# knagrecha/saturn

Hardware: AMD Instinct MI355X
Metric: samples_per_s (higher is better)
Workload: dtype bf16; 1 GPU; model=gptj-6b, global_batch=16, seq_len=512, parallelism=dp1, optimizer=fused_sgd

## Files before the change

### saturn_amd/executors/megatron.py

```python

from __future__ import annotations

from timeit import default_timer as timer
from typing import Any, Dict, List, Optional, Tuple

from saturn_amd.core.technique import BaseTechnique
from saturn_amd.executors.launch import (
    destroy_process_group,
    gang_spawn,
    init_process_group,
)

TRIAL_BATCHES = 3


def _tp_worker(rank: int, world: int, task, tid: int, batch_count: int,
               params: Optional[Dict[str, Any]], trial: bool):
    import torch
    import torch.distributed as dist

    from saturn_amd.executors.ddp import _make_optimizer
    from saturn_amd.parallel.tensor import (
        tp_full_state_dict,
        tp_resync_replicated,
        tp_shard_model,
    )

    backend = init_process_group(rank, world)
    try:
        device = (
            torch.device("cuda", rank) if backend == "nccl" else torch.device("cpu")
        )
        dtype = torch.bfloat16 if backend == "nccl" else torch.float32
        from saturn_amd.executors.ddp import build_model_on

        model = build_model_on(task, device, dtype)
        model.train()
        if world > 1:
            with torch.no_grad():
                for p in model.parameters():
                    dist.broadcast(p.data, src=0)
        model = tp_shard_model(model)
        optimizer = _make_optimizer(task, model)

        import os as _os

        opt_path = _os.path.join(
            task.save_dir, f"{task.name}.tpopt.w{world}.r{rank}.pt"
        )
        if not trial and _os.path.isfile(opt_path):
            try:
                optimizer.load_state_dict(
                    torch.load(opt_path, map_location="cpu", weights_only=False)
                )
            except Exception:
                pass

        it = task.get_iterator() if not trial else task.get_fresh_iterator()

        def next_batch():
            nonlocal it
            try:
                return next(it)
            except StopIteration:
                it = task.get_fresh_iterator()
                return next(it)

        def step(batch):
            x, y = batch
            x = x.to(device, non_blocking=True)
            y = y.to(device, non_blocking=True)
            if x.is_floating_point():
                x = x.to(dtype)
            loss = task.loss_function(model(x), y)
            loss.backward()
            optimizer.step()
            optimizer.zero_grad(set_to_none=True)

        if trial:
            step(next_batch())
            if device.type == "cuda":
                torch.cuda.synchronize()
                torch.cuda.reset_peak_memory_stats()
            t0 = timer()
            for _ in range(TRIAL_BATCHES - 1):
                step(next_batch())
            if device.type == "cuda":
                torch.cuda.synchronize()
            hbm = (
                torch.cuda.max_memory_allocated() / 2**30
                if device.type == "cuda"
                else 0.0
            )
            return ((timer() - t0) / (TRIAL_BATCHES - 1), hbm)
        RESYNC_EVERY = 64
        for i in range(batch_count):
            step(next_batch())
            if (i + 1) % RESYNC_EVERY == 0:
                tp_resync_replicated(model)
        if device.type == "cuda":
            torch.cuda.synchronize()
        tp_resync_replicated(model)
        sd = tp_full_state_dict(model)
        if rank == 0 and sd is not None:
            task.save_checkpoint(sd, None)
        if _os.environ.get("SATURN_SKIP_CKPT") != "1":
            tmp = opt_path + ".tmp"
            torch.save(optimizer.state_dict(), tmp)
            _os.replace(tmp, opt_path)
        if world > 1:
            dist.barrier()
        return None
    finally:
        destroy_process_group()


class MegatronExecutor(BaseTechnique):

    name = "megatron"

    @staticmethod
    def execute(task, gpus: List[int], tid: int, batch_count: int) -> None:
        params = (
            task.selected_strategy.parameters
            if task.selected_strategy is not None
            else {}
        )
        gang_spawn(_tp_worker, len(gpus), tid, task, tid, batch_count, params, False)

    @staticmethod
    def search(
        task, gpus: List[int], tid: int
    ) -> Tuple[Optional[Dict[str, Any]], float]:
        if len(gpus) < 2:
            return None, float("inf")
        try:
            out = gang_spawn(
                _tp_worker, len(gpus), tid, task, tid, TRIAL_BATCHES,
                {"tp": len(gpus)}, True,
            )
        except Exception:
            return None, float("inf")
        if out is None:
            return None, float("inf")
        bt, hbm = out
        return dict(tp=len(gpus), hbm_peak_gb=round(hbm, 2)), bt
```

### saturn_amd/models/gptj.py

```python

from __future__ import annotations


import os
from dataclasses import dataclass

import torch
import torch.nn as nn

from saturn_amd.ops.functional import (
    fused_gelu,
    FusedLayerNorm,
    apply_rope,
    causal_attention,
    fused_add3,
    fused_cross_entropy,
    rope_tables,
    FusedDropout,
    FusedEmbedding,
    gptj_mlp,
    mlp_fused_supported,
    gptj_branches,
    gptj_branches_supported,
)


@dataclass
class GPTJConfig:
    vocab_size: int = 50400
    n_ctx: int = 512
    n_embd: int = 4096
    n_head: int = 16
    n_layer: int = 28
    rotary_dim: int = 64
    embd_pdrop: float = 0.0
    resid_pdrop: float = 0.0


class GPTJAttention(nn.Module):
    def __init__(self, cfg: GPTJConfig):
        super().__init__()
        self.n_head = cfg.n_head
        self.head_dim = cfg.n_embd // cfg.n_head
        self.rotary_dim = cfg.rotary_dim
        E = cfg.n_embd
        self.q_proj = nn.Linear(E, E, bias=False)
        self.k_proj = nn.Linear(E, E, bias=False)
        self.v_proj = nn.Linear(E, E, bias=False)
        self.out_proj = nn.Linear(E, E, bias=False)
        self.n_ctx = cfg.n_ctx
        self._rope_f32 = rope_tables(cfg.n_ctx, cfg.rotary_dim)

    def _rope(self, device):
        if self._rope_f32[0].device != device:
            self._rope_f32 = tuple(t.to(device) for t in self._rope_f32)
        return self._rope_f32

    def forward(self, x):
        B, T, E = x.shape
        H, D = self.n_head, self.head_dim
        q = self.q_proj(x).view(B, T, H, D)
        k = self.k_proj(x).view(B, T, H, D)
        v = self.v_proj(x).view(B, T, H, D)
        cos, sin = self._rope(x.device)
        q = apply_rope(q, cos, sin)
        k = apply_rope(k, cos, sin)
        q = q.transpose(1, 2)
        k = k.transpose(1, 2)
        v = v.transpose(1, 2)
        o = causal_attention(q, k, v)
        o = o.transpose(1, 2).reshape(B, T, -1)
        return self.out_proj(o)


class GPTJMLP(nn.Module):
    def __init__(self, cfg: GPTJConfig):
        super().__init__()
        E = cfg.n_embd
        self.fc_in = nn.Linear(E, 4 * E)
        self.fc_out = nn.Linear(4 * E, E)

    @staticmethod
    def _plain_linear(m) -> bool:
        return type(m) is nn.Linear and not (
            m._forward_hooks
            or m._forward_pre_hooks
            or m._backward_hooks
            or m._backward_pre_hooks
        )

    def _use_fused(self, x) -> bool:
        if os.environ.get("SAMD_MLP_FUSED", "1") == "0":
            return False
        fi, fo = self.fc_in, self.fc_out
        return (
            x.is_cuda
            and self._plain_linear(fi)
            and self._plain_linear(fo)
            and mlp_fused_supported(x, fi.weight, fi.bias, fo.weight, fo.bias)
        )

    def forward(self, x):
        if self._use_fused(x):
            fi, fo = self.fc_in, self.fc_out
            return gptj_mlp(x, fi.weight, fi.bias, fo.weight, fo.bias)
        return self.fc_out(fused_gelu(self.fc_in(x)))


class GPTJBlock(nn.Module):

    def __init__(self, cfg: GPTJConfig):
        super().__init__()
        self.ln_1 = FusedLayerNorm(cfg.n_embd)
        self.attn = GPTJAttention(cfg)
        self.mlp = GPTJMLP(cfg)
        self.drop = FusedDropout(cfg.resid_pdrop)

    @staticmethod
    def _hooked(m) -> bool:
        return bool(
            m._forward_hooks
            or m._forward_pre_hooks
            or m._backward_hooks
            or m._backward_pre_hooks
        )

    def _use_fused(self, h) -> bool:
        if (os.environ.get("SAMD_MLP_FUSED", "1") == "0"
                or os.environ.get("SAMD_BLOCK_FUSED", "1") == "0"):
            return False
        attn, mlp = self.attn, self.mlp
        if type(attn) is not GPTJAttention or type(mlp) is not GPTJMLP:
            return False
        if not (h.is_cuda and h.dtype == torch.bfloat16 and h.dim() == 3):
            return False
        if self.drop.p != 0.0:
            return False
        from saturn_amd.parallel.sequence import sp_world

        if sp_world() != 1:
            return False
        if any(self._hooked(m) for b in (attn, mlp, self.drop) for m in b.modules()):
            return False
        projs = (attn.q_proj, attn.k_proj, attn.v_proj, attn.out_proj)
        fi, fo = mlp.fc_in, mlp.fc_out
        if not all(GPTJMLP._plain_linear(m) for m in (*projs, fi, fo)):
            return False
        E = h.shape[-1]
        if any(m.bias is not None or m.weight.shape != (E, E)
               or m.weight.dtype != torch.bfloat16 or not m.weight.is_cuda
               for m in projs):
            return False
        return mlp_fused_supported(
            h, fi.weight, fi.bias, fo.weight, fo.bias
        ) and gptj_branches_supported(
            h, attn.n_head, attn.rotary_dim, attn._rope_f32[0].shape[0]
        )

    def forward(self, x):
        h = self.ln_1(x)
        if self._use_fused(h):
            attn, mlp = self.attn, self.mlp
            cos, sin = attn._rope(h.device)
            a, m = gptj_branches(
                h, attn.q_proj.weight, attn.k_proj.weight, attn.v_proj.weight,
                attn.out_proj.weight, mlp.fc_in.weight, mlp.fc_in.bias,
                mlp.fc_out.weight, mlp.fc_out.bias, cos, sin, attn.n_head,
            )
            return fused_add3(x, a, m)
        return fused_add3(x, self.drop(self.attn(h)), self.drop(self.mlp(h)))


class GPTJForCausalLM(nn.Module):
    def __init__(self, cfg: GPTJConfig):
        super().__init__()
        self.cfg = cfg
        self.wte = FusedEmbedding(cfg.vocab_size, cfg.n_embd)
        self.drop = FusedDropout(cfg.embd_pdrop)
        self.h = nn.ModuleList(GPTJBlock(cfg) for _ in range(cfg.n_layer))
        self.ln_f = FusedLayerNorm(cfg.n_embd)
        self.lm_head = nn.Linear(cfg.n_embd, cfg.vocab_size, bias=True)
        self.apply(self._init)

    @staticmethod
    def _init(m):
        if isinstance(m, nn.Linear):
            nn.init.normal_(m.weight, std=0.02)
            if m.bias is not None:
                nn.init.zeros_(m.bias)
        elif isinstance(m, nn.Embedding):
            nn.init.normal_(m.weight, std=0.02)

    def forward(self, input_ids):
        x = self.drop(self.wte(input_ids))
        for block in self.h:
            x = block(x)
        x = self.ln_f(x)
        return self.lm_head(x)


def pretraining_loss(logits, labels):
    return fused_cross_entropy(logits, labels, shift=True)


class _EmbedStage(nn.Module):
    def __init__(self, wte):
        super().__init__()
        self.wte = wte

    def forward(self, input_ids):
        return self.wte(input_ids)


class _HeadStage(nn.Module):
    def __init__(self, ln_f, lm_head):
        super().__init__()
        self.ln_f = ln_f
        self.lm_head = lm_head

    def forward(self, x):
        return self.lm_head(self.ln_f(x))


def as_sequential(model: GPTJForCausalLM) -> nn.Sequential:
    return nn.Sequential(
        _EmbedStage(model.wte), *model.h, _HeadStage(model.ln_f, model.lm_head)
    )


def get_gptj_model(kwargs=None):
    kwargs = kwargs or {}
    cfg = GPTJConfig(
        n_layer=kwargs.get("n_layer", 28),
        n_embd=kwargs.get("n_embd", 4096),
        n_head=kwargs.get("n_head", 16),
        n_ctx=kwargs.get("n_ctx", 512),
        vocab_size=kwargs.get("vocab_size", 50400),
        rotary_dim=kwargs.get("rotary_dim", 64),
        embd_pdrop=kwargs.get("embd_pdrop", 0.0),
        resid_pdrop=kwargs.get("resid_pdrop", 0.0),
    )
    torch.manual_seed(kwargs.get("seed", 0))
    return GPTJForCausalLM(cfg)


class SyntheticTokens(torch.utils.data.Dataset):

    def __init__(self, n: int, seq_len: int, vocab: int, seed: int = 1):
        g = torch.Generator().manual_seed(seed)
        self.data = torch.randint(0, vocab, (n, seq_len), generator=g)

    def __len__(self):
        return len(self.data)

    def __getitem__(self, i):
        return self.data[i]


def _collate(batch):
    x = torch.stack(batch)
    return x, x.clone()


def make_token_dataloader(batch_size=8, seq_len=512, vocab=50400, n_batches=64):
    def get_dataloader():
        return torch.utils.data.DataLoader(
            SyntheticTokens(batch_size * n_batches, seq_len, vocab),
            batch_size=batch_size,
            shuffle=False,
            collate_fn=_collate,
        )

    return get_dataloader
```

### saturn_amd/ops/csrc/bindings.cpp

```cpp

#include <torch/extension.h>
#include <vector>

namespace samd {
void fused_sgd(std::vector<at::Tensor> params, std::vector<at::Tensor> grads,
               std::vector<at::Tensor> moms, std::vector<at::Tensor> masters,
               double lr, double momentum, double weight_decay);
void fused_adam(std::vector<at::Tensor> params, std::vector<at::Tensor> grads,
                std::vector<at::Tensor> ms, std::vector<at::Tensor> vs,
                std::vector<at::Tensor> masters, double lr, double beta1,
                double beta2, double eps, double weight_decay, double bc1,
                double bc2);
std::vector<at::Tensor> norm_fwd(at::Tensor x, at::Tensor w,
                                 c10::optional<at::Tensor> b, double eps,
                                 bool rms);
std::vector<at::Tensor> norm_bwd(at::Tensor dy, at::Tensor x, at::Tensor w,
                                 at::Tensor mean, at::Tensor rstd, bool rms,
                                 bool needs_db);
std::vector<at::Tensor> ce_fwd(at::Tensor logits, at::Tensor targets,
                               int64_t Tr, int64_t ignore_index);
at::Tensor ce_bwd(at::Tensor logits, at::Tensor targets, at::Tensor lse,
                  at::Tensor dloss, int64_t Tr, int64_t ignore_index);
void rope_apply(at::Tensor y, at::Tensor x, at::Tensor cos_t, at::Tensor sin_t,
                int64_t t_len, int64_t t_off, bool half_style, bool backward);
at::Tensor gelu_fwd(at::Tensor x);
at::Tensor gelu_bwd(at::Tensor dy, at::Tensor x);
std::vector<at::Tensor> attn_fwd(at::Tensor q, at::Tensor k, at::Tensor v,
                                 bool causal, int64_t kv_len);
std::vector<at::Tensor> attn_bwd(at::Tensor dout, at::Tensor q, at::Tensor k,
                                 at::Tensor v, at::Tensor o, at::Tensor lse,
                                 bool causal, int64_t kv_len);
std::string attn_dispatch(int64_t T, int64_t D);
at::Tensor add3(at::Tensor a, at::Tensor b, at::Tensor c);
at::Tensor swiglu_fwd(at::Tensor gate, at::Tensor up);
std::vector<at::Tensor> swiglu_bwd(at::Tensor dout, at::Tensor gate,
                                   at::Tensor up);
at::Tensor embed_fwd(at::Tensor weight, at::Tensor idx);
at::Tensor embed_bwd(at::Tensor dout, at::Tensor idx, long vocab);
at::Tensor dropout_fwd(at::Tensor x, double p, long seed);
at::Tensor dropout_bwd(at::Tensor dout, double p, long seed);
std::vector<at::Tensor> moe_route_fwd(at::Tensor logits, int64_t top_k,
                                      at::ScalarType out_dtype);
at::Tensor moe_route_bwd(at::Tensor logits, at::Tensor ids,
                         at::Tensor dweights);
std::vector<at::Tensor> moe_sort(at::Tensor ids, int64_t n_expert);
at::Tensor moe_permute_fwd(at::Tensor x, at::Tensor order, int64_t top_k);
at::Tensor moe_permute_bwd(at::Tensor dxs, at::Tensor pos);
at::Tensor moe_combine_fwd(at::Tensor y, at::Tensor weights, at::Tensor pos);
std::vector<at::Tensor> moe_combine_bwd(at::Tensor dout, at::Tensor y,
                                        at::Tensor weights, at::Tensor pos);
std::vector<at::Tensor> mlp_act_bwd(at::Tensor d_act, at::Tensor pre,
                                    bool want_dT, bool want_aT);
std::vector<at::Tensor> transpose_colsum(at::Tensor x, bool want_sum);
std::vector<at::Tensor> mlp_bwd(at::Tensor g, at::Tensor h, at::Tensor pre,
                                at::Tensor W_in, at::Tensor W_out,
                                bool use_tn_in, bool use_tn_out);
void transpose_into(at::Tensor x, at::Tensor dst);
at::Tensor rope_bwd_t(at::Tensor dy, at::Tensor cos_t, at::Tensor sin_t,
                      int64_t t_len, int64_t t_off, int64_t dim,
                      at::Tensor dxT);
std::vector<at::Tensor> gptj_branches_bwd(
    at::Tensor g_a, at::Tensor g_m, at::Tensor h, at::Tensor pre, at::Tensor q,
    at::Tensor k, at::Tensor v, at::Tensor o, at::Tensor lse, at::Tensor Wq,
    at::Tensor Wk, at::Tensor Wv, at::Tensor Wo, at::Tensor W_in,
    at::Tensor W_out, at::Tensor cos_t, at::Tensor sin_t, int64_t t_off,
    bool tn_in, bool tn_out, bool tn_qkv, bool tn_o, bool dh_accum);
}

PYBIND11_MODULE(TORCH_EXTENSION_NAME, m) {
  m.doc() = "saturn_amd hand-written CDNA4 (gfx950) kernels";
  m.def("fused_sgd", &samd::fused_sgd, "fused multi-tensor SGD");
  m.def("fused_adam", &samd::fused_adam, "fused multi-tensor AdamW");
  m.def("norm_fwd", &samd::norm_fwd, "LayerNorm/RMSNorm forward");
  m.def("norm_bwd", &samd::norm_bwd, "LayerNorm/RMSNorm backward");
  m.def("ce_fwd", &samd::ce_fwd, "fused cross-entropy forward");
  m.def("ce_bwd", &samd::ce_bwd, "fused cross-entropy backward");
  m.def("rope_apply", &samd::rope_apply,
        "fused rotary embedding (out-of-place, offset table rows)");
  m.def("gelu_fwd", &samd::gelu_fwd, "fused tanh-approx GELU forward");
  m.def("gelu_bwd", &samd::gelu_bwd, "fused tanh-approx GELU backward");
  m.def("attn_fwd", &samd::attn_fwd, "fused flash attention forward",
        py::arg("q"), py::arg("k"), py::arg("v"), py::arg("causal"),
        py::arg("kv_len") = -1);
  m.def("attn_dispatch", &samd::attn_dispatch,
        "kernel instantiations attn_fwd/attn_bwd launch for (padded T, D)",
        py::arg("T"), py::arg("D"));
  m.def("attn_bwd", &samd::attn_bwd, "fused flash attention backward",
        py::arg("dout"), py::arg("q"), py::arg("k"), py::arg("v"),
        py::arg("o"), py::arg("lse"), py::arg("causal"),
        py::arg("kv_len") = -1);
  m.def("add3", &samd::add3, "fused 3-way residual add");
  m.def("swiglu_fwd", &samd::swiglu_fwd, "fused silu(gate)*up");
  m.def("swiglu_bwd", &samd::swiglu_bwd, "fused SwiGLU backward");
  m.def("embed_fwd", &samd::embed_fwd, "token embedding gather");
  m.def("embed_bwd", &samd::embed_bwd, "embedding scatter-add backward");
  m.def("dropout_fwd", &samd::dropout_fwd, "counter-based fused dropout");
  m.def("dropout_bwd", &samd::dropout_bwd, "dropout backward (mask recompute)");
  m.def("moe_route_fwd", &samd::moe_route_fwd,
        "MoE softmax + top-k + renormalise (ties to the lower expert)");
  m.def("moe_route_bwd", &samd::moe_route_bwd, "MoE routing backward");
  m.def("moe_sort", &samd::moe_sort,
        "stable counting sort of (token, slot) pairs by expert");
  m.def("moe_permute_fwd", &samd::moe_permute_fwd,
        "gather token rows into expert order");
  m.def("moe_permute_bwd", &samd::moe_permute_bwd,
        "sum each token's k permuted rows");
  m.def("moe_combine_fwd", &samd::moe_combine_fwd,
        "weighted sum of each token's k expert rows");
  m.def("moe_combine_bwd", &samd::moe_combine_bwd,
        "combine backward: dy and fp32 dweights");
  m.def("mlp_act_bwd", &samd::mlp_act_bwd,
        "GELU backward + transposed d_pre / gelu(pre) + fp32 bias grad",
        py::arg("d_act"), py::arg("pre"), py::arg("want_dT") = true,
        py::arg("want_aT") = true);
  m.def("transpose_colsum", &samd::transpose_colsum,
        "bf16 transpose with optional fp32 column sums");
  m.def("mlp_bwd", &samd::mlp_bwd,
        "GPT-J MLP backward with TN-layout weight gradients");
  m.def("transpose_into", &samd::transpose_into,
        "bf16 transpose stored into a caller-given [N, M] view",
        py::arg("x"), py::arg("dst"));
  m.def("rope_bwd_t", &samd::rope_bwd_t,
        "interleaved RoPE backward that also stores dx^T into a [E, M] view",
        py::arg("dy"), py::arg("cos"), py::arg("sin"), py::arg("t_len"),
        py::arg("t_off"), py::arg("dim"), py::arg("dxT"));
  m.def("gptj_branches_bwd", &samd::gptj_branches_bwd,
        "GPT-J attention + MLP branch backward with shared transposes");
}
```

### saturn_amd/ops/csrc/fused_optim.hip

```cpp

#include <torch/extension.h>
#include <ATen/hip/HIPContext.h>
#include <vector>

#include "common.h"

namespace samd {

constexpr int MAX_T = 32;
constexpr int GRP = 8;

typedef __attribute__((ext_vector_type(8))) short short8v_;
typedef __attribute__((ext_vector_type(4))) float float4v_;

struct SgdArgs {
  void* p[MAX_T];
  void* g[MAX_T];
  void* m[MAX_T];
  void* w[MAX_T];
  long cum[MAX_T + 1];
  long numel[MAX_T];
  int n_tensors;
  float lr, momentum, weight_decay;
};

template <typename T, bool HAS_M, bool HAS_W>
__device__ __forceinline__ void sgd_elem(T* p, const T* g, float* m, float* w,
                                         long j, const SgdArgs& a) {
  float pv = HAS_W ? w[j] : toF<T>(p[j]);
  float gv = toF<T>(g[j]);
  if (a.weight_decay != 0.f) gv += a.weight_decay * pv;
  if (HAS_M) {
    float mv = m[j] * a.momentum + gv;
    m[j] = mv;
    gv = mv;
  }
  float nv = pv - a.lr * gv;
  if (HAS_W) w[j] = nv;
  p[j] = fromF<T>(nv);
}

template <typename T, bool HAS_M, bool HAS_W>
__global__ void fused_sgd_kernel(SgdArgs a) {
  const long total = a.cum[a.n_tensors];
  const long stride = (long)gridDim.x * blockDim.x;
  for (long i = blockIdx.x * (long)blockDim.x + threadIdx.x; i < total;
       i += stride) {
    int t = 0;
#pragma unroll
    for (int k = 0; k < MAX_T; ++k)
      if (k < a.n_tensors && i >= a.cum[k + 1]) t = k + 1;
    const long grp = i - a.cum[t];
    const long base = grp * GRP;
    T* p = reinterpret_cast<T*>(a.p[t]);
    const T* g = reinterpret_cast<const T*>(a.g[t]);
    float* m = HAS_M ? reinterpret_cast<float*>(a.m[t]) : nullptr;
    float* w = HAS_W ? reinterpret_cast<float*>(a.w[t]) : nullptr;
    const long n = a.numel[t];
    if constexpr (sizeof(T) == 2) {
      if (base + GRP <= n) {
        short8v_ pv = *reinterpret_cast<short8v_*>(p + base);
        short8v_ gv = *reinterpret_cast<const short8v_*>(g + base);
        float4v_ m0, m1, w0, w1;
        if (HAS_M) {
          m0 = *reinterpret_cast<float4v_*>(m + base);
          m1 = *reinterpret_cast<float4v_*>(m + base + 4);
        }
        if (HAS_W) {
          w0 = *reinterpret_cast<float4v_*>(w + base);
          w1 = *reinterpret_cast<float4v_*>(w + base + 4);
        }
#pragma unroll
        for (int e = 0; e < GRP; ++e) {
          T pe, ge;
          pe.x = (unsigned short)pv[e];
          ge.x = (unsigned short)gv[e];
          float pf = HAS_W ? (e < 4 ? w0[e] : w1[e - 4]) : toF<T>(pe);
          float gf = toF<T>(ge);
          if (a.weight_decay != 0.f) gf += a.weight_decay * pf;
          if (HAS_M) {
            float mv = (e < 4 ? m0[e] : m1[e - 4]) * a.momentum + gf;
            if (e < 4) m0[e] = mv; else m1[e - 4] = mv;
            gf = mv;
          }
          float nf = pf - a.lr * gf;
          if (HAS_W) {
            if (e < 4) w0[e] = nf; else w1[e - 4] = nf;
          }
          T out = fromF<T>(nf);
          pv[e] = (short)out.x;
        }
        *reinterpret_cast<short8v_*>(p + base) = pv;
        if (HAS_M) {
          *reinterpret_cast<float4v_*>(m + base) = m0;
          *reinterpret_cast<float4v_*>(m + base + 4) = m1;
        }
        if (HAS_W) {
          *reinterpret_cast<float4v_*>(w + base) = w0;
          *reinterpret_cast<float4v_*>(w + base + 4) = w1;
        }
      } else {
        for (long j = base; j < n; ++j)
          sgd_elem<T, HAS_M, HAS_W>(p, g, m, w, j, a);
      }
    } else {
      const long end = (base + GRP <= n) ? base + GRP : n;
      for (long j = base; j < end; ++j)
        sgd_elem<T, HAS_M, HAS_W>(p, g, m, w, j, a);
    }
  }
}

struct AdamArgs {
  void* p[MAX_T];
  void* g[MAX_T];
  void* m[MAX_T];
  void* v[MAX_T];
  void* w[MAX_T];
  long cum[MAX_T + 1];
  long numel[MAX_T];
  int n_tensors;
  float lr, beta1, beta2, eps, weight_decay, bc1, bc2;
};

template <typename T, bool HAS_W>
__device__ __forceinline__ void adam_elem(T* p, const T* g, float* m, float* v,
                                          float* w, long j, const AdamArgs& a,
                                          float inv_bc1, float inv_bc2) {
  float gv = toF<T>(g[j]);
  float mv = a.beta1 * m[j] + (1.f - a.beta1) * gv;
  float vv = a.beta2 * v[j] + (1.f - a.beta2) * gv * gv;
  m[j] = mv;
  v[j] = vv;
  float denom = sqrtf(vv * inv_bc2) + a.eps;
  float upd = (mv * inv_bc1) / denom;
  float pv = HAS_W ? w[j] : toF<T>(p[j]);
  if (a.weight_decay != 0.f) pv *= (1.f - a.lr * a.weight_decay);
  float nv = pv - a.lr * upd;
  if (HAS_W) w[j] = nv;
  p[j] = fromF<T>(nv);
}

template <typename T, bool HAS_W>
__global__ void fused_adam_kernel(AdamArgs a) {
  const long total = a.cum[a.n_tensors];
  const long stride = (long)gridDim.x * blockDim.x;
  const float inv_bc1 = 1.f / a.bc1;
  const float inv_bc2 = 1.f / a.bc2;
  for (long i = blockIdx.x * (long)blockDim.x + threadIdx.x; i < total;
       i += stride) {
    int t = 0;
#pragma unroll
    for (int k = 0; k < MAX_T; ++k)
      if (k < a.n_tensors && i >= a.cum[k + 1]) t = k + 1;
    const long grp = i - a.cum[t];
    const long base = grp * GRP;
    T* p = reinterpret_cast<T*>(a.p[t]);
    const T* g = reinterpret_cast<const T*>(a.g[t]);
    float* m = reinterpret_cast<float*>(a.m[t]);
    float* v = reinterpret_cast<float*>(a.v[t]);
    float* w = HAS_W ? reinterpret_cast<float*>(a.w[t]) : nullptr;
    const long n = a.numel[t];
    if constexpr (sizeof(T) == 2) {
      if (base + GRP <= n) {
        short8v_ pv = *reinterpret_cast<short8v_*>(p + base);
        short8v_ gv = *reinterpret_cast<const short8v_*>(g + base);
        float4v_ m0 = *reinterpret_cast<float4v_*>(m + base);
        float4v_ m1 = *reinterpret_cast<float4v_*>(m + base + 4);
        float4v_ v0 = *reinterpret_cast<float4v_*>(v + base);
        float4v_ v1 = *reinterpret_cast<float4v_*>(v + base + 4);
        float4v_ w0, w1;
        if (HAS_W) {
          w0 = *reinterpret_cast<float4v_*>(w + base);
          w1 = *reinterpret_cast<float4v_*>(w + base + 4);
        }
#pragma unroll
        for (int e = 0; e < GRP; ++e) {
          T ge;
          ge.x = (unsigned short)gv[e];
          float gf = toF<T>(ge);
          float mv = a.beta1 * (e < 4 ? m0[e] : m1[e - 4]) + (1.f - a.beta1) * gf;
          float vv = a.beta2 * (e < 4 ? v0[e] : v1[e - 4]) + (1.f - a.beta2) * gf * gf;
          if (e < 4) { m0[e] = mv; v0[e] = vv; } else { m1[e-4] = mv; v1[e-4] = vv; }
          float denom = sqrtf(vv * inv_bc2) + a.eps;
          float upd = (mv * inv_bc1) / denom;
          T pe;
          pe.x = (unsigned short)pv[e];
          float pf = HAS_W ? (e < 4 ? w0[e] : w1[e - 4]) : toF<T>(pe);
          if (a.weight_decay != 0.f) pf *= (1.f - a.lr * a.weight_decay);
          float nf = pf - a.lr * upd;
          if (HAS_W) {
            if (e < 4) w0[e] = nf; else w1[e - 4] = nf;
          }
          T out = fromF<T>(nf);
          pv[e] = (short)out.x;
        }
        *reinterpret_cast<short8v_*>(p + base) = pv;
        *reinterpret_cast<float4v_*>(m + base) = m0;
        *reinterpret_cast<float4v_*>(m + base + 4) = m1;
        *reinterpret_cast<float4v_*>(v + base) = v0;
        *reinterpret_cast<float4v_*>(v + base + 4) = v1;
        if (HAS_W) {
          *reinterpret_cast<float4v_*>(w + base) = w0;
          *reinterpret_cast<float4v_*>(w + base + 4) = w1;
        }
      } else {
        for (long j = base; j < n; ++j)
          adam_elem<T, HAS_W>(p, g, m, v, w, j, a, inv_bc1, inv_bc2);
      }
    } else {
      const long end = (base + GRP <= n) ? base + GRP : n;
      for (long j = base; j < end; ++j)
        adam_elem<T, HAS_W>(p, g, m, v, w, j, a, inv_bc1, inv_bc2);
    }
  }
}

static int grid_for(long total, int block) {
  long g = (total + block - 1) / block;
  return (int)std::min<long>(std::max<long>(g, 1), 4096);
}

static long groups_of(long numel) { return (numel + GRP - 1) / GRP; }

template <typename scalar_t>
static void sgd_launch(std::vector<at::Tensor>& params,
                       std::vector<at::Tensor>& grads,
                       std::vector<at::Tensor>& moms,
                       std::vector<at::Tensor>& masters, double lr,
                       double momentum, double weight_decay) {
  auto stream = at::hip::getCurrentHIPStream();
  const bool has_m = !moms.empty();
  const bool has_w = !masters.empty();
  for (size_t base = 0; base < params.size(); base += MAX_T) {
    SgdArgs a{};
    a.n_tensors = (int)std::min<size_t>(MAX_T, params.size() - base);
    a.lr = (float)lr;
    a.momentum = (float)momentum;
    a.weight_decay = (float)weight_decay;
    long cum = 0;
    a.cum[0] = 0;
    for (int k = 0; k < a.n_tensors; ++k) {
      a.p[k] = params[base + k].data_ptr();
      a.g[k] = grads[base + k].data_ptr();
      a.m[k] = has_m ? moms[base + k].data_ptr() : nullptr;
      a.w[k] = has_w ? masters[base + k].data_ptr() : nullptr;
      a.numel[k] = params[base + k].numel();
      cum += groups_of(a.numel[k]);
      a.cum[k + 1] = cum;
    }
    const int block = 256;
    dim3 grid(grid_for(cum, block));
    if (has_m && has_w)
      hipLaunchKernelGGL((fused_sgd_kernel<scalar_t, true, true>), grid,
                         dim3(block), 0, stream.stream(), a);
    else if (has_m)
      hipLaunchKernelGGL((fused_sgd_kernel<scalar_t, true, false>), grid,
                         dim3(block), 0, stream.stream(), a);
    else if (has_w)
      hipLaunchKernelGGL((fused_sgd_kernel<scalar_t, false, true>), grid,
                         dim3(block), 0, stream.stream(), a);
    else
      hipLaunchKernelGGL((fused_sgd_kernel<scalar_t, false, false>), grid,
                         dim3(block), 0, stream.stream(), a);
  }
}

void fused_sgd(std::vector<at::Tensor> params, std::vector<at::Tensor> grads,
               std::vector<at::Tensor> moms, std::vector<at::Tensor> masters,
               double lr, double momentum, double weight_decay) {
  TORCH_CHECK(!params.empty(), "no params");
  TORCH_CHECK(params.size() == grads.size());
  TORCH_CHECK(moms.empty() || moms.size() == params.size());
  TORCH_CHECK(masters.empty() || masters.size() == params.size());
  for (size_t i = 0; i < params.size(); ++i) {
    TORCH_CHECK(params[i].is_contiguous() && grads[i].is_contiguous());
    TORCH_CHECK(params[i].scalar_type() == grads[i].scalar_type());
    if (!moms.empty())
      TORCH_CHECK(moms[i].scalar_type() == at::kFloat,
                  "momentum buffers must be fp32");
    if (!masters.empty())
      TORCH_CHECK(masters[i].scalar_type() == at::kFloat &&
                      masters[i].is_contiguous(),
                  "master weights must be contiguous fp32");
  }
  switch (params[0].scalar_type()) {
    case at::kBFloat16:
      sgd_launch<c10::BFloat16>(params, grads, moms, masters, lr, momentum,
                                weight_decay);
      break;
    case at::kFloat:
      sgd_launch<float>(params, grads, moms, masters, lr, momentum,
                        weight_decay);
      break;
    case at::kHalf:
      sgd_launch<c10::Half>(params, grads, moms, masters, lr, momentum,
                            weight_decay);
      break;
    default:
      TORCH_CHECK(false, "fused_sgd: unsupported dtype");
  }
}

template <typename scalar_t>
static void adam_launch(std::vector<at::Tensor>& params,
                        std::vector<at::Tensor>& grads,
                        std::vector<at::Tensor>& ms,
                        std::vector<at::Tensor>& vs,
                        std::vector<at::Tensor>& masters, double lr,
                        double beta1, double beta2, double eps,
                        double weight_decay, double bc1, double bc2) {
  auto stream = at::hip::getCurrentHIPStream();
  const bool has_w = !masters.empty();
  for (size_t base = 0; base < params.size(); base += MAX_T) {
    AdamArgs a{};
    a.n_tensors = (int)std::min<size_t>(MAX_T, params.size() - base);
    a.lr = (float)lr;
    a.beta1 = (float)beta1;
    a.beta2 = (float)beta2;
    a.eps = (float)eps;
    a.weight_decay = (float)weight_decay;
    a.bc1 = (float)bc1;
    a.bc2 = (float)bc2;
    long cum = 0;
    a.cum[0] = 0;
    for (int k = 0; k < a.n_tensors; ++k) {
      a.p[k] = params[base + k].data_ptr();
      a.g[k] = grads[base + k].data_ptr();
      a.m[k] = ms[base + k].data_ptr();
      a.v[k] = vs[base + k].data_ptr();
      a.w[k] = has_w ? masters[base + k].data_ptr() : nullptr;
      a.numel[k] = params[base + k].numel();
      cum += groups_of(a.numel[k]);
      a.cum[k + 1] = cum;
    }
    const int block = 256;
    dim3 grid(grid_for(cum, block));
    if (has_w)
      hipLaunchKernelGGL((fused_adam_kernel<scalar_t, true>), grid,
                         dim3(block), 0, stream.stream(), a);
    else
      hipLaunchKernelGGL((fused_adam_kernel<scalar_t, false>), grid,
                         dim3(block), 0, stream.stream(), a);
  }
}

void fused_adam(std::vector<at::Tensor> params, std::vector<at::Tensor> grads,
                std::vector<at::Tensor> ms, std::vector<at::Tensor> vs,
                std::vector<at::Tensor> masters, double lr, double beta1,
                double beta2, double eps, double weight_decay, double bc1,
                double bc2) {
  TORCH_CHECK(!params.empty(), "no params");
  TORCH_CHECK(params.size() == grads.size() && params.size() == ms.size() &&
              params.size() == vs.size());
  TORCH_CHECK(masters.empty() || masters.size() == params.size());
  for (size_t i = 0; i < params.size(); ++i) {
    TORCH_CHECK(params[i].is_contiguous() && grads[i].is_contiguous());
    TORCH_CHECK(ms[i].scalar_type() == at::kFloat &&
                vs[i].scalar_type() == at::kFloat,
                "Adam moments must be fp32");
    if (!masters.empty())
      TORCH_CHECK(masters[i].scalar_type() == at::kFloat &&
                      masters[i].is_contiguous(),
                  "master weights must be contiguous fp32");
  }
  switch (params[0].scalar_type()) {
    case at::kBFloat16:
      adam_launch<c10::BFloat16>(params, grads, ms, vs, masters, lr, beta1,
                                 beta2, eps, weight_decay, bc1, bc2);
      break;
    case at::kFloat:
      adam_launch<float>(params, grads, ms, vs, masters, lr, beta1, beta2,
                         eps, weight_decay, bc1, bc2);
      break;
    default:
      TORCH_CHECK(false, "fused_adam: unsupported dtype");
  }
}

}
```

### saturn_amd/ops/csrc/gptj_block_bwd.hip

```cpp

#include <torch/extension.h>
#include <ATen/hip/HIPContext.h>

#include "common.h"
#include "tile_image.h"

namespace samd {

std::vector<at::Tensor> attn_bwd(at::Tensor dout, at::Tensor q, at::Tensor k,
                                 at::Tensor v, at::Tensor o, at::Tensor lse,
                                 bool causal, int64_t kv_len);
std::vector<at::Tensor> mlp_act_bwd(at::Tensor d_act, at::Tensor pre,
                                    bool want_dT, bool want_aT);
void rope_apply(at::Tensor y, at::Tensor x, at::Tensor cos_t, at::Tensor sin_t,
                int64_t t_len, int64_t t_off, bool half_style, bool backward);

namespace {

__global__ void __launch_bounds__(MB_BLOCK)
rope_bwd_t_kernel(const bf16_t* __restrict__ dy, bf16_t* __restrict__ dx,
                  bf16_t* __restrict__ dxT, const float* __restrict__ cos_t,
                  const float* __restrict__ sin_t, long M, long E, int t_len,
                  long t_off, int dim, int half, float sign) {
  __shared__ uint4 img[MB_TILE * 8];

  const int tid = threadIdx.x;
  const int cv = tid & 7;
  const int rp = tid >> 3;
  const int mv = tid & 7;
  const int cr = tid >> 3;
  const long col0 = (long)blockIdx.x * MB_TILE;
  const long col = col0 + cv * 8;
  const bool col_ok = col < E;
  const int j0 = (int)(col % dim);
  const bool rotary = j0 < 2 * half;

  for (int it = 0; it < MB_ROW_ITERS; ++it) {
    const long row0 = ((long)blockIdx.y * MB_ROW_ITERS + it) * MB_TILE;
    if (row0 >= M) break;
    const long row = row0 + 2 * rp;
    const bool ok = col_ok && row < M;

    const short8v zero8 = {0, 0, 0, 0, 0, 0, 0, 0};
    short8v ov[2];
#pragma unroll
    for (int i = 0; i < 2; ++i) {
      ov[i] = zero8;
      if (!ok) continue;
      const short8v xv =
          *reinterpret_cast<const short8v*>(dy + (row + i) * E + col);
      if (rotary) {
        const long trow = (t_off + ((row + i) % t_len)) * (long)half;
#pragma unroll
        for (int e = 0; e < 4; ++e) {
          const int p = j0 / 2 + e;
          const float c = cos_t[trow + p];
          const float s = sin_t[trow + p] * sign;
          bf16_t e0, e1;
          e0.x = (unsigned short)xv[2 * e];
          e1.x = (unsigned short)xv[2 * e + 1];
          const float x0 = toF<bf16_t>(e0);
          const float x1 = toF<bf16_t>(e1);
          ov[i][2 * e] = (short)fromF<bf16_t>(x0 * c - x1 * s).x;
          ov[i][2 * e + 1] = (short)fromF<bf16_t>(x1 * c + x0 * s).x;
        }
      } else {
        ov[i] = xv;
      }
      *reinterpret_cast<short8v*>(dx + (row + i) * E + col) = ov[i];
    }
    unsigned* i32 = reinterpret_cast<unsigned*>(img);
#pragma unroll
    for (int e = 0; e < 8; ++e) {
      i32[img_dword(cv * 8 + e, rp)] =
          (unsigned)(unsigned short)ov[0][e] |
          ((unsigned)(unsigned short)ov[1][e] << 16);
    }
    __syncthreads();

    const long mrow = row0 + mv * 8;
#pragma unroll
    for (int j = 0; j < 2; ++j) {
      const int c = cr + 32 * j;
      if ((col0 + c < E) && (mrow < M))
        *reinterpret_cast<uint4*>(dxT + (col0 + c) * M + mrow) =
            img[img_slot(c, mv)];
    }
    __syncthreads();
  }
}

void check_f32_table(const at::Tensor& t, const char* name) {
  TORCH_CHECK(t.is_cuda() && t.scalar_type() == at::kFloat && t.dim() == 2 &&
                  t.is_contiguous(),
              name, ": expected a contiguous fp32 [T, half] GPU tensor");
}

}

at::Tensor rope_bwd_t(at::Tensor dy, at::Tensor cos_t, at::Tensor sin_t,
                      int64_t t_len, int64_t t_off, int64_t dim,
                      at::Tensor dxT) {
  TORCH_CHECK(dy.is_cuda() && dy.scalar_type() == at::kBFloat16 &&
                  dy.is_contiguous() && dy.numel() > 0,
              "rope_bwd_t dy: expected a contiguous bf16 GPU tensor");
  check_f32_table(cos_t, "rope_bwd_t cos");
  check_f32_table(sin_t, "rope_bwd_t sin");
  const long half = cos_t.size(1);
  TORCH_CHECK(sin_t.sizes() == cos_t.sizes(), "rope_bwd_t: table mismatch");
  TORCH_CHECK(dim > 0 && dim % 8 == 0, "rope_bwd_t: head dim ", dim,
              " must be a positive multiple of 8");
  TORCH_CHECK((2 * half) % 8 == 0 && 2 * half <= dim,
              "rope_bwd_t: rotary dim ", 2 * half,
              " must be a multiple of 8 within the head dim");
  TORCH_CHECK(dy.numel() % dim == 0 && dy.size(-1) == dim,
              "rope_bwd_t: last dim of dy must be the head dim");
  TORCH_CHECK(dy.dim() >= 2, "rope_bwd_t dy: expected [..., heads, dim]");
  const long E = dy.size(-2) * dim;
  const long M = dy.numel() / E;
  TORCH_CHECK(M % 8 == 0, "rope_bwd_t: token count ", M,
              " must be a multiple of 8");
  TORCH_CHECK(t_len > 0 && M % t_len == 0,
              "rope_bwd_t: token count not a multiple of T");
  TORCH_CHECK(t_off >= 0 && cos_t.size(0) >= t_off + t_len,
              "rope_bwd_t: table too short for offset+T");
  TORCH_CHECK(reinterpret_cast<uintptr_t>(dy.data_ptr()) % 16 == 0,
              "rope_bwd_t dy: data must be 16-byte aligned");
  check_operand(dxT, "rope_bwd_t dxT");
  TORCH_CHECK(dxT.size(0) == E && dxT.size(1) == M &&
                  dxT.device() == dy.device(),
              "rope_bwd_t: dxT must be [", E, ", ", M, "], got ", dxT.sizes());

  auto dx = at::empty_like(dy);
  const dim3 grid = tile_grid(M, E);
  auto stream = at::hip::getCurrentHIPStream();
  hipLaunchKernelGGL(rope_bwd_t_kernel, grid, dim3(MB_BLOCK), 0,
                     stream.stream(), bptr(dy), bptr(dx), bptr(dxT),
                     cos_t.data_ptr<float>(), sin_t.data_ptr<float>(), M, E,
                     (int)t_len, (long)t_off, (int)dim, (int)half, -1.f);
  SAMD_CHECK_HIP(hipGetLastError());
  return dx;
}

std::vector<at::Tensor> gptj_branches_bwd(
    at::Tensor g_a, at::Tensor g_m, at::Tensor h, at::Tensor pre, at::Tensor q,
    at::Tensor k, at::Tensor v, at::Tensor o, at::Tensor lse, at::Tensor Wq,
    at::Tensor Wk, at::Tensor Wv, at::Tensor Wo, at::Tensor W_in,
    at::Tensor W_out, at::Tensor cos_t, at::Tensor sin_t, int64_t t_off,
    bool tn_in, bool tn_out, bool tn_qkv, bool tn_o, bool dh_accum) {
  check_operand(g_a, "gptj_branches_bwd g_a");
  check_operand(g_m, "gptj_branches_bwd g_m");
  check_operand(h, "gptj_branches_bwd h");
  check_operand(pre, "gptj_branches_bwd pre");
  check_operand(W_in, "gptj_branches_bwd W_in");
  check_operand(W_out, "gptj_branches_bwd W_out");
  const long M = h.size(0), E = h.size(1), F = pre.size(1);
  TORCH_CHECK(q.dim() == 4 && o.dim() == 4, "gptj_branches_bwd: q, o 4-D");
  const long B = q.size(0), H = q.size(1), T = q.size(2), D = q.size(3);
  TORCH_CHECK(B * T == M && H * D == E && k.sizes() == q.sizes() &&
                  v.sizes() == q.sizes() && o.sizes() == q.sizes(),
              "gptj_branches_bwd: attention shapes do not match h");
  TORCH_CHECK(g_a.sizes() == h.sizes() && g_m.sizes() == h.sizes() &&
                  pre.size(0) == M && W_in.size(0) == F && W_in.size(1) == E &&
                  W_out.size(0) == E && W_out.size(1) == F,
              "gptj_branches_bwd: inconsistent shapes");
  for (const at::Tensor* w : {&Wq, &Wk, &Wv, &Wo}) {
    check_operand(*w, "gptj_branches_bwd projection weight");
    TORCH_CHECK(w->size(0) == E && w->size(1) == E,
                "gptj_branches_bwd: projection weights must be [E, E]");
  }
  auto o_phys = o.permute({0, 2, 1, 3});
  TORCH_CHECK(o_phys.is_contiguous(),
              "gptj_branches_bwd: o must be physically [B,T,H,D]");
  auto o2 = o_phys.view({M, E});
  const bool shared = g_a.data_ptr() == g_m.data_ptr();

  auto gt = transpose_colsum_impl(g_m, true, tn_out || (shared && tn_o));
  at::Tensor gaT;
  if (tn_o) gaT = shared ? gt[0] : transpose_colsum_impl(g_a, false, true)[0];
  at::Tensor hT;
  if (tn_in || tn_qkv) hT = transpose_colsum_impl(h, false, true)[0];

  at::Tensor dh, dW_in, db_in, dW_out;
  {
    at::Tensor d_pre, d_preT, act;
    {
      auto d_act = at::mm(g_m, W_out);
      auto r = mlp_act_bwd(d_act, pre, tn_in, tn_out);
      d_pre = r[0];
      d_preT = r[1];
      act = r[2];
      db_in = r[3];
    }
    dW_out = tn_out ? at::linear(gt[0], act) : at::mm(g_m.t(), act);
    act.reset();
    if (!tn_o) gt[0].reset();
    dW_in = tn_in ? at::linear(d_preT, hT) : at::mm(d_pre.t(), h);
    d_preT.reset();
    if (!tn_qkv) hT.reset();
    dh = at::mm(d_pre, W_in);
  }

  auto d_o = at::mm(g_a, Wo);
  at::Tensor dWo;
  if (tn_o) {
    auto oT = transpose_colsum_impl(o2, false, true)[0];
    dWo = at::linear(gaT, oT);
    gaT.reset();
    gt[0].reset();
  } else {
    dWo = at::mm(g_a.t(), o2);
  }

  at::Tensor dq_r, dk_r, dv;
  {
    auto r = attn_bwd(d_o.view({B, T, H, D}).permute({0, 2, 1, 3}), q, k, v, o,
                      lse, true, T);
    dq_r = r[0].permute({0, 2, 1, 3});
    dk_r = r[1].permute({0, 2, 1, 3});
    dv = r[2].permute({0, 2, 1, 3});
    TORCH_CHECK(dq_r.is_contiguous() && dk_r.is_contiguous() &&
                    dv.is_contiguous(),
                "gptj_branches_bwd: attn_bwd layout changed");
  }
  d_o.reset();
  auto dv2 = dv.view({M, E});

  at::Tensor dq, dk, dWq, dWk, dWv;
  if (tn_qkv) {
    auto dqkvT = at::empty({3 * E, M}, h.options());
    dq = rope_bwd_t(dq_r, cos_t, sin_t, T, t_off, D, dqkvT.narrow(0, 0, E));
    dq_r.reset();
    dk = rope_bwd_t(dk_r, cos_t, sin_t, T, t_off, D, dqkvT.narrow(0, E, E));
    dk_r.reset();
    transpose_colsum_impl(dv2, false, true, dqkvT.narrow(0, 2 * E, E));
    auto dW = at::linear(dqkvT, hT);
    dqkvT.reset();
    hT.reset();
    dWq = dW.narrow(0, 0, E);
    dWk = dW.narrow(0, E, E);
    dWv = dW.narrow(0, 2 * E, E);
  } else {
    dq = at::empty_like(dq_r);
    rope_apply(dq, dq_r, cos_t, sin_t, T, t_off, false, true);
    dq_r.reset();
    dk = at::empty_like(dk_r);
    rope_apply(dk, dk_r, cos_t, sin_t, T, t_off, false, true);
    dk_r.reset();
    dWq = at::mm(dq.view({M, E}).t(), h);
    dWk = at::mm(dk.view({M, E}).t(), h);
    dWv = at::mm(dv2.t(), h);
  }

  auto dq2 = dq.view({M, E}), dk2 = dk.view({M, E});
  if (dh_accum) {
    dh.addmm_(dv2, Wv);
    dh.addmm_(dk2, Wk);
    dh.addmm_(dq2, Wq);
  } else {
    dh.add_(at::mm(dv2, Wv));
    dh.add_(at::mm(dk2, Wk));
    dh.add_(at::mm(dq2, Wq));
  }
  return {dh, dWq, dWk, dWv, dWo, dW_in, db_in.to(W_in.scalar_type()),
          dW_out, gt[1].to(W_out.scalar_type())};
}

}
```

### saturn_amd/ops/csrc/mlp_bwd.hip

```cpp

#include <torch/extension.h>
#include <ATen/hip/HIPContext.h>

#include "common.h"
#include "gelu_math.h"
#include "tile_image.h"

namespace samd {

namespace {

template <bool TN_IN, bool TN_OUT>
__global__ void __launch_bounds__(MB_BLOCK)
mlp_act_bwd_kernel(const bf16_t* __restrict__ d_act,
                   const bf16_t* __restrict__ pre, bf16_t* __restrict__ d_pre,
                   bf16_t* __restrict__ d_preT, bf16_t* __restrict__ act,
                   float* __restrict__ partial, long M, long F) {
  __shared__ uint4 img_d[MB_TILE * 8];
  __shared__ uint4 img_a[TN_OUT ? MB_TILE * 8 : 1];
  __shared__ float4 lds_sum[MB_TILE / 4];

  const int tid = threadIdx.x;
  const int cv = tid & 7;
  const int rp = tid >> 3;
  const int mv = tid & 7;
  const int cr = tid >> 3;
  const long col0 = (long)blockIdx.x * MB_TILE;
  const long col = col0 + cv * 8;
  const bool col_ok = col < F;

  float acc0 = 0.f, acc1 = 0.f;

  for (int it = 0; it < MB_ROW_ITERS; ++it) {
    const long row0 = ((long)blockIdx.y * MB_ROW_ITERS + it) * MB_TILE;
    if (row0 >= M) break;
    const long row = row0 + 2 * rp;
    const bool ok = col_ok && row < M;

    const short8v zero8 = {0, 0, 0, 0, 0, 0, 0, 0};
    short8v xv[2], gv[2];
#pragma unroll
    for (int i = 0; i < 2; ++i) {
      if (ok) {
        const long o = (row + i) * F + col;
        xv[i] = *reinterpret_cast<const short8v*>(pre + o);
        gv[i] = *reinterpret_cast<const short8v*>(d_act + o);
      } else {
        xv[i] = zero8;
        gv[i] = zero8;
      }
    }
    short8v dv[2], av[2];
#pragma unroll
    for (int i = 0; i < 2; ++i) {
#pragma unroll
      for (int e = 0; e < 8; ++e) {
        bf16_t xe, de;
        xe.x = (unsigned short)xv[i][e];
        de.x = (unsigned short)gv[i][e];
        const float xf = toF<bf16_t>(xe);
        dv[i][e] = (short)fromF<bf16_t>(toF<bf16_t>(de) * dgelu_f(xf)).x;
        av[i][e] = (short)fromF<bf16_t>(gelu_f(xf)).x;
      }
    }
    if (ok) {
#pragma unroll
      for (int i = 0; i < 2; ++i) {
        const long o = (row + i) * F + col;
        *reinterpret_cast<short8v*>(d_pre + o) = dv[i];
        if (!TN_OUT) *reinterpret_cast<short8v*>(act + o) = av[i];
      }
    }
    unsigned* d32 = reinterpret_cast<unsigned*>(img_d);
    unsigned* a32 = reinterpret_cast<unsigned*>(img_a);
#pragma unroll
    for (int e = 0; e < 8; ++e) {
      const int w = img_dword(cv * 8 + e, rp);
      d32[w] = ok ? ((unsigned)(unsigned short)dv[0][e] |
                     ((unsigned)(unsigned short)dv[1][e] << 16))
                  : 0u;
      if (TN_OUT)
        a32[w] = ok ? ((unsigned)(unsigned short)av[0][e] |
                       ((unsigned)(unsigned short)av[1][e] << 16))
                    : 0u;
    }
    __syncthreads();

    const long mrow = row0 + mv * 8;
#pragma unroll
    for (int j = 0; j < 2; ++j) {
      const int c = cr + 32 * j;
      const uint4 d = img_d[img_slot(c, mv)];
      const float s = sum8_bf16(d);
      if (j == 0) acc0 += s; else acc1 += s;
      const bool st = (col0 + c < F) && (mrow < M);
      if (TN_IN && st)
        *reinterpret_cast<uint4*>(d_preT + (col0 + c) * M + mrow) = d;
      if (TN_OUT && st)
        *reinterpret_cast<uint4*>(act + (col0 + c) * M + mrow) =
            img_a[img_slot(c, mv)];
    }
    __syncthreads();
  }
  store_colsums(acc0, acc1, lds_sum, partial, col0, F);
}

template <bool SUM, bool STORE>
__global__ void __launch_bounds__(MB_BLOCK)
transpose_colsum_kernel(const bf16_t* __restrict__ x, bf16_t* __restrict__ xT,
                        float* __restrict__ partial, long M, long N) {
  __shared__ uint4 img[MB_TILE * 8];
  __shared__ float4 lds_sum[MB_TILE / 4];

  const int tid = threadIdx.x;
  const int cv = tid & 7;
  const int rp = tid >> 3;
  const int mv = tid & 7;
  const int cr = tid >> 3;
  const long col0 = (long)blockIdx.x * MB_TILE;
  const long col = col0 + cv * 8;
  const bool col_ok = col < N;

  float acc0 = 0.f, acc1 = 0.f;

  for (int it = 0; it < MB_ROW_ITERS; ++it) {
    const long row0 = ((long)blockIdx.y * MB_ROW_ITERS + it) * MB_TILE;
    if (row0 >= M) break;
    const long row = row0 + 2 * rp;
    const bool ok = col_ok && row < M;

    const short8v zero8 = {0, 0, 0, 0, 0, 0, 0, 0};
    short8v xv[2];
#pragma unroll
    for (int i = 0; i < 2; ++i) {
      xv[i] = zero8;
      if (ok) xv[i] = *reinterpret_cast<const short8v*>(x + (row + i) * N + col);
    }
    unsigned* i32 = reinterpret_cast<unsigned*>(img);
#pragma unroll
    for (int e = 0; e < 8; ++e) {
      i32[img_dword(cv * 8 + e, rp)] =
          (unsigned)(unsigned short)xv[0][e] |
          ((unsigned)(unsigned short)xv[1][e] << 16);
    }
    __syncthreads();

    const long mrow = row0 + mv * 8;
#pragma unroll
    for (int j = 0; j < 2; ++j) {
      const int c = cr + 32 * j;
      const uint4 v = img[img_slot(c, mv)];
      if (SUM) {
        const float s = sum8_bf16(v);
        if (j == 0) acc0 += s; else acc1 += s;
      }
      if (STORE && (col0 + c < N) && (mrow < M))
        *reinterpret_cast<uint4*>(xT + (col0 + c) * M + mrow) = v;
    }
    __syncthreads();
  }
  if (SUM) store_colsums(acc0, acc1, lds_sum, partial, col0, N);
}

}

std::vector<at::Tensor> mlp_act_bwd(at::Tensor d_act, at::Tensor pre,
                                    bool want_dT, bool want_aT) {
  check_operand(d_act, "mlp_act_bwd d_act");
  check_operand(pre, "mlp_act_bwd pre");
  TORCH_CHECK(d_act.sizes() == pre.sizes(), "mlp_act_bwd: shape mismatch");
  const long M = pre.size(0), F = pre.size(1);
  auto d_pre = at::empty_like(pre);
  auto d_preT = want_dT ? at::empty({F, M}, pre.options())
                        : at::empty({0}, pre.options());
  auto act = want_aT ? at::empty({F, M}, pre.options()) : at::empty_like(pre);
  const dim3 grid = tile_grid(M, F);
  auto partial =
      at::empty({(long)grid.y, F}, pre.options().dtype(at::kFloat));
  auto stream = at::hip::getCurrentHIPStream();
#define SAMD_LAUNCH_ACT_BWD(TI, TO)                                        \
  hipLaunchKernelGGL((mlp_act_bwd_kernel<TI, TO>), grid, dim3(MB_BLOCK), 0, \
                     stream.stream(), bptr(d_act), bptr(pre), bptr(d_pre),  \
                     want_dT ? bptr(d_preT) : nullptr, bptr(act),           \
                     partial.data_ptr<float>(), M, F)
  if (want_dT && want_aT) SAMD_LAUNCH_ACT_BWD(true, true);
  else if (want_dT) SAMD_LAUNCH_ACT_BWD(true, false);
  else if (want_aT) SAMD_LAUNCH_ACT_BWD(false, true);
  else SAMD_LAUNCH_ACT_BWD(false, false);
#undef SAMD_LAUNCH_ACT_BWD
  SAMD_CHECK_HIP(hipGetLastError());
  return {d_pre, d_preT, act, at::sum(partial, {0})};
}

std::vector<at::Tensor> transpose_colsum_impl(
    const at::Tensor& x, bool want_sum, bool want_store,
    const c10::optional<at::Tensor>& dst) {
  check_operand(x, "transpose_colsum x");
  TORCH_CHECK(want_sum || want_store, "transpose_colsum: nothing to do");
  const long M = x.size(0), N = x.size(1);
  at::Tensor xT;
  if (want_store && dst.has_value()) {
    xT = *dst;
    check_operand(xT, "transpose_colsum dst");
    TORCH_CHECK(xT.size(0) == N && xT.size(1) == M &&
                    xT.device() == x.device(),
                "transpose_colsum: dst must be [", N, ", ", M, "], got ",
                xT.sizes());
  } else {
    xT = want_store ? at::empty({N, M}, x.options())
                    : at::empty({0}, x.options());
  }
  const dim3 grid = tile_grid(M, N);
  const auto fopt = x.options().dtype(at::kFloat);
  auto partial = want_sum ? at::empty({(long)grid.y, N}, fopt)
                          : at::empty({0}, fopt);
  auto stream = at::hip::getCurrentHIPStream();
#define SAMD_LAUNCH_TRANSPOSE(SUM, STORE)                                    \
  hipLaunchKernelGGL((transpose_colsum_kernel<SUM, STORE>), grid,            \
                     dim3(MB_BLOCK), 0, stream.stream(), bptr(x),            \
                     want_store ? bptr(xT) : nullptr,                        \
                     want_sum ? partial.data_ptr<float>() : nullptr, M, N)
  if (want_sum && want_store) SAMD_LAUNCH_TRANSPOSE(true, true);
  else if (want_sum) SAMD_LAUNCH_TRANSPOSE(true, false);
  else SAMD_LAUNCH_TRANSPOSE(false, true);
#undef SAMD_LAUNCH_TRANSPOSE
  SAMD_CHECK_HIP(hipGetLastError());
  return {xT, want_sum ? at::sum(partial, {0}) : partial};
}

std::vector<at::Tensor> transpose_colsum(at::Tensor x, bool want_sum) {
  return transpose_colsum_impl(x, want_sum, true);
}

void transpose_into(at::Tensor x, at::Tensor dst) {
  transpose_colsum_impl(x, false, true, dst);
}

std::vector<at::Tensor> mlp_bwd(at::Tensor g, at::Tensor h, at::Tensor pre,
                                at::Tensor W_in, at::Tensor W_out,
                                bool use_tn_in, bool use_tn_out) {
  check_operand(g, "mlp_bwd g");
  check_operand(h, "mlp_bwd h");
  check_operand(pre, "mlp_bwd pre");
  check_operand(W_in, "mlp_bwd W_in");
  check_operand(W_out, "mlp_bwd W_out");
  const long M = g.size(0), E = g.size(1), F = pre.size(1);
  TORCH_CHECK(h.size(0) == M && h.size(1) == E && pre.size(0) == M &&
                  W_in.size(0) == F && W_in.size(1) == E &&
                  W_out.size(0) == E && W_out.size(1) == F,
              "mlp_bwd: inconsistent shapes");

  at::Tensor d_pre, d_preT, act, db_in;
  {
    auto d_act = at::mm(g, W_out);
    auto r = mlp_act_bwd(d_act, pre, use_tn_in, use_tn_out);
    d_pre = r[0];
    d_preT = r[1];
    act = r[2];
    db_in = r[3];
  }
  auto gt = transpose_colsum_impl(g, true, use_tn_out);
  at::Tensor hT;
  if (use_tn_in) hT = transpose_colsum_impl(h, false, true)[0];
  auto dW_out = use_tn_out ? at::linear(gt[0], act) : at::mm(g.t(), act);
  act.reset();
  auto dW_in = use_tn_in ? at::linear(d_preT, hT) : at::mm(d_pre.t(), h);
  d_preT.reset();
  hT.reset();
  auto dh = at::mm(d_pre, W_in);
  return {dh, dW_in, db_in.to(W_in.scalar_type()), dW_out,
          gt[1].to(W_out.scalar_type())};
}

}
```

### saturn_amd/ops/csrc/tile_image.h

```cpp
#pragma once

#include <torch/extension.h>

#include <vector>

#include "common.h"

namespace samd {

constexpr int MB_TILE = 64;
constexpr int MB_ROW_ITERS = 4;
constexpr int MB_BLOCK = 256;

typedef c10::BFloat16 bf16_t;

__device__ __forceinline__ int img_dword(int c, int rp) {
  return c * 32 + (((rp >> 2) ^ (c >> 3)) << 2) + (rp & 3);
}
__device__ __forceinline__ int img_slot(int c, int mv) {
  return c * 8 + (mv ^ (c >> 3));
}

__device__ __forceinline__ float sum8_bf16(const uint4 v) {
  float s = us2f((unsigned short)(v.x & 0xffffu));
  s += us2f((unsigned short)(v.x >> 16));
  s += us2f((unsigned short)(v.y & 0xffffu));
  s += us2f((unsigned short)(v.y >> 16));
  s += us2f((unsigned short)(v.z & 0xffffu));
  s += us2f((unsigned short)(v.z >> 16));
  s += us2f((unsigned short)(v.w & 0xffffu));
  s += us2f((unsigned short)(v.w >> 16));
  return s;
}

__device__ __forceinline__ void store_colsums(float acc0, float acc1,
                                              float4* lds_sum,
                                              float* __restrict__ partial,
                                              long col0, long ncols) {
  const int tid = threadIdx.x;
#pragma unroll
  for (int off = 1; off < 8; off <<= 1) {
    acc0 += __shfl_xor(acc0, off, 64);
    acc1 += __shfl_xor(acc1, off, 64);
  }
  float* s = reinterpret_cast<float*>(lds_sum);
  if ((tid & 7) == 0) {
    s[tid >> 3] = acc0;
    s[(tid >> 3) + 32] = acc1;
  }
  __syncthreads();
  if (tid < MB_TILE / 4 && col0 + tid * 4 < ncols) {
    *reinterpret_cast<float4*>(partial + (long)blockIdx.y * ncols + col0 +
                               tid * 4) = lds_sum[tid];
  }
}

inline void check_operand(const at::Tensor& t, const char* name) {
  TORCH_CHECK(t.is_cuda(), name, ": expected a GPU tensor");
  TORCH_CHECK(t.scalar_type() == at::kBFloat16, name, ": expected bf16");
  TORCH_CHECK(t.dim() == 2 && t.is_contiguous(), name,
              ": expected a contiguous 2-D tensor");
  TORCH_CHECK(t.size(0) > 0 && t.size(0) % 8 == 0 && t.size(1) > 0 &&
                  t.size(1) % 8 == 0,
              name, ": both sizes must be positive multiples of 8, got ",
              t.sizes());
  TORCH_CHECK(reinterpret_cast<uintptr_t>(t.data_ptr()) % 16 == 0, name,
              ": data must be 16-byte aligned");
}

inline dim3 tile_grid(long M, long N) {
  const long gx = (N + MB_TILE - 1) / MB_TILE;
  const long gy = (M + MB_TILE * MB_ROW_ITERS - 1) / (MB_TILE * MB_ROW_ITERS);
  TORCH_CHECK(gy <= 65535, "mlp_bwd: too many rows for one launch");
  return dim3((unsigned)gx, (unsigned)gy);
}

inline bf16_t* bptr(const at::Tensor& t) {
  return reinterpret_cast<bf16_t*>(t.data_ptr());
}

std::vector<at::Tensor> transpose_colsum_impl(
    const at::Tensor& x, bool want_sum, bool want_store,
    const c10::optional<at::Tensor>& dst = c10::nullopt);

}
```

### saturn_amd/ops/functional.py

```python

from __future__ import annotations

import os
from typing import Tuple

import torch
import torch.nn.functional as F

from saturn_amd.ops import require_ext


class _NormFn(torch.autograd.Function):
    @staticmethod
    def forward(ctx, x, w, b, eps, rms):
        ext = require_ext()
        x = x.contiguous()
        y, mean, rstd = ext.norm_fwd(x, w, b, eps, rms)
        if rms:
            mean = rstd
        ctx.save_for_backward(x, w, mean, rstd)
        ctx.rms = rms
        ctx.has_b = b is not None
        return y

    @staticmethod
    def backward(ctx, dy):
        ext = require_ext()
        x, w, mean, rstd = ctx.saved_tensors
        dx, dw, db = ext.norm_bwd(
            dy.contiguous(), x, w, mean, rstd, ctx.rms, ctx.has_b
        )
        return (
            dx,
            dw.to(w.dtype),
            db.to(w.dtype) if ctx.has_b else None,
            None,
            None,
        )


def fused_layer_norm(x, weight, bias=None, eps: float = 1e-5):
    if x.is_cuda:
        return _NormFn.apply(x, weight, bias, eps, False)
    return F.layer_norm(
        x.float(), (x.shape[-1],),
        weight.float(), bias.float() if bias is not None else None, eps
    ).to(x.dtype)


def fused_rms_norm(x, weight, eps: float = 1e-6):
    if x.is_cuda:
        return _NormFn.apply(x, weight, None, eps, True)
    xf = x.float()
    y = xf * torch.rsqrt(xf.pow(2).mean(-1, keepdim=True) + eps)
    return (y * weight.float()).to(x.dtype)


class FusedLayerNorm(torch.nn.Module):
    def __init__(self, dim: int, eps: float = 1e-5, bias: bool = True):
        super().__init__()
        self.eps = eps
        self.weight = torch.nn.Parameter(torch.ones(dim))
        self.bias = torch.nn.Parameter(torch.zeros(dim)) if bias else None

    def forward(self, x):
        return fused_layer_norm(x, self.weight, self.bias, self.eps)


class FusedRMSNorm(torch.nn.Module):
    def __init__(self, dim: int, eps: float = 1e-6):
        super().__init__()
        self.eps = eps
        self.weight = torch.nn.Parameter(torch.ones(dim))

    def forward(self, x):
        return fused_rms_norm(x, self.weight, self.eps)


class _CeFn(torch.autograd.Function):
    @staticmethod
    def forward(ctx, logits, targets_flat, Tr, ignore_index):
        ext = require_ext()
        loss, lse = ext.ce_fwd(logits, targets_flat, Tr, ignore_index)
        valid = (targets_flat != ignore_index).sum().clamp(min=1)
        ctx.save_for_backward(logits, targets_flat, lse, valid)
        ctx.Tr = Tr
        ctx.ignore_index = ignore_index
        return loss.sum() / valid.float()

    @staticmethod
    def backward(ctx, grad_out):
        ext = require_ext()
        logits, targets_flat, lse, valid = ctx.saved_tensors
        dloss = torch.full_like(lse, 0.0)
        dloss.fill_(1.0)
        dloss = dloss * (grad_out.float() / valid.float())
        dlogits = ext.ce_bwd(
            logits, targets_flat, lse, dloss, ctx.Tr, ctx.ignore_index
        )
        return dlogits, None, None, None


def fused_cross_entropy(
    logits: torch.Tensor,
    targets: torch.Tensor,
    shift: bool = True,
    ignore_index: int = -100,
) -> torch.Tensor:
    B, T, V = logits.shape
    if logits.is_cuda:
        Tr = T - 1 if shift else T
        tg = targets[:, 1:] if shift else targets
        return _CeFn.apply(
            logits.contiguous(), tg.contiguous().view(-1), Tr, ignore_index
        )
    if shift:
        lg = logits[:, :-1].float().reshape(-1, V)
        tg = targets[:, 1:].reshape(-1)
    else:
        lg = logits.float().reshape(-1, V)
        tg = targets.reshape(-1)
    return F.cross_entropy(lg, tg, ignore_index=ignore_index)


def rope_tables(
    T: int,
    rotary_dim: int,
    base: float = 10000.0,
    device=None,
    interleaved: bool = True,
) -> Tuple[torch.Tensor, torch.Tensor]:
    half = rotary_dim // 2
    inv = 1.0 / (base ** (torch.arange(0, half, dtype=torch.float32) * 2 / rotary_dim))
    t = torch.arange(T, dtype=torch.float32)
    freqs = torch.outer(t, inv)
    return freqs.cos().to(device), freqs.sin().to(device)


class _RopeFn(torch.autograd.Function):
    @staticmethod
    def forward(ctx, x, cos_t, sin_t, t_len, t_off, half_style):
        ext = require_ext()
        x = x.contiguous()
        y = torch.empty_like(x)
        ext.rope_apply(y, x, cos_t, sin_t, t_len, t_off, half_style, False)
        ctx.save_for_backward(cos_t, sin_t)
        ctx.meta = (t_len, t_off, half_style)
        return y

    @staticmethod
    def backward(ctx, dy):
        ext = require_ext()
        cos_t, sin_t = ctx.saved_tensors
        t_len, t_off, half_style = ctx.meta
        dy = dy.contiguous()
        dx = torch.empty_like(dy)
        ext.rope_apply(dx, dy, cos_t, sin_t, t_len, t_off, half_style, True)
        return dx, None, None, None, None, None


def _rope_cpu(x, cos_bt, sin_bt, half_style):
    B, T, H, D = x.shape
    half = cos_bt.shape[-1]
    c = cos_bt.view(B, T, 1, half).float()
    s = sin_bt.view(B, T, 1, half).float()
    xf = x.float()
    out = xf.clone()
    if half_style:
        x0 = xf[..., :half]
        x1 = xf[..., half : 2 * half]
        out[..., :half] = x0 * c - x1 * s
        out[..., half : 2 * half] = x1 * c + x0 * s
    else:
        x0 = xf[..., 0 : 2 * half : 2]
        x1 = xf[..., 1 : 2 * half : 2]
        out[..., 0 : 2 * half : 2] = x0 * c - x1 * s
        out[..., 1 : 2 * half : 2] = x1 * c + x0 * s
    return out.to(x.dtype)


def apply_rope(
    x: torch.Tensor,
    cos: torch.Tensor,
    sin: torch.Tensor,
    half_style: bool = False,
) -> torch.Tensor:
    B, T, H, D = x.shape
    half = cos.shape[-1]
    from saturn_amd.parallel.sequence import _STATE as _sp

    off = _sp["rank"] * T if _sp["world"] > 1 else 0
    if cos.shape[0] < off + T:
        raise ValueError(
            "rope table too short for this sequence shard — pass the FULL "
            "table to apply_rope (it slices positions itself)"
        )
    if cos.dtype != torch.float32:
        cos = cos.float()
        sin = sin.float()
    if x.is_cuda:
        return _RopeFn.apply(x, cos.contiguous(), sin.contiguous(), T, off,
                             half_style)
    cos_bt = cos[off : off + T].unsqueeze(0).expand(B, T, half)
    sin_bt = sin[off : off + T].unsqueeze(0).expand(B, T, half)
    return _rope_cpu(x, cos_bt.contiguous(), sin_bt.contiguous(), half_style)


def attention_math(q, k, v, causal: bool = True) -> torch.Tensor:
    scale = 1.0 / (q.shape[-1] ** 0.5)
    s = torch.matmul(q.float(), k.float().transpose(-1, -2)) * scale
    if causal:
        T = q.shape[-2]
        mask = torch.ones(T, T, dtype=torch.bool, device=q.device).tril()
        s = s.masked_fill(~mask, float("-inf"))
    p = torch.softmax(s, dim=-1)
    return torch.matmul(p, v.float()).to(q.dtype)


def _attention_core(q, k, v, causal: bool) -> torch.Tensor:
    if q.is_cuda:
        from saturn_amd.ops import flash

        return flash.flash_attention(q, k, v, causal=causal)
    if k.shape[1] != q.shape[1]:
        rep = q.shape[1] // k.shape[1]
        k = k.repeat_interleave(rep, dim=1)
        v = v.repeat_interleave(rep, dim=1)
    return attention_math(q, k, v, causal=causal)


def _attention(q, k, v, causal: bool) -> torch.Tensor:
    from saturn_amd.parallel.sequence import sp_attention, sp_world

    if sp_world() > 1:
        return sp_attention(q, k, v, lambda a, b, c: _attention_core(a, b, c, causal))
    return _attention_core(q, k, v, causal)


def causal_attention(q, k, v) -> torch.Tensor:
    return _attention(q, k, v, causal=True)


def full_attention(q, k, v) -> torch.Tensor:
    return _attention(q, k, v, causal=False)


class _Add3Fn(torch.autograd.Function):
    @staticmethod
    def forward(ctx, a, b, c):
        ext = require_ext()
        return ext.add3(a.contiguous(), b.contiguous(), c.contiguous())

    @staticmethod
    def backward(ctx, g):
        return g, g, g


def fused_add3(a, b, c):
    if a.is_cuda:
        return _Add3Fn.apply(a, b, c)
    return a + b + c


class _GeluFn(torch.autograd.Function):
    @staticmethod
    def forward(ctx, x):
        ext = require_ext()
        x = x.contiguous()
        ctx.save_for_backward(x)
        return ext.gelu_fwd(x)

    @staticmethod
    def backward(ctx, dy):
        ext = require_ext()
        (x,) = ctx.saved_tensors
        return ext.gelu_bwd(dy.contiguous(), x)


def fused_gelu(x: torch.Tensor) -> torch.Tensor:
    if x.is_cuda and x.dtype in (torch.bfloat16, torch.float16):
        return _GeluFn.apply(x)
    return torch.nn.functional.gelu(x, approximate="tanh")


_MLP_TN_DEFAULT = {"in": True, "out": True}


def _mlp_tn(site: str) -> bool:
    v = os.environ.get("SAMD_MLP_TN_" + site.upper())
    return _MLP_TN_DEFAULT[site] if v is None else v != "0"


def mlp_fused_supported(x, w_in, b_in, w_out, b_out) -> bool:
    if not (x.is_cuda and x.dtype == torch.bfloat16 and x.dim() >= 2):
        return False
    if b_in is None or b_out is None:
        return False
    if any(t.dtype != torch.bfloat16 or not t.is_cuda
           for t in (w_in, b_in, w_out, b_out)):
        return False
    E = x.shape[-1]
    M = x.numel() // E if E else 0
    F_ = w_in.shape[0]
    return (
        M > 0
        and w_in.shape == (F_, E)
        and w_out.shape == (E, F_)
        and M % 8 == 0
        and E % 8 == 0
        and F_ % 8 == 0
    )


class _GPTJMlpFn(torch.autograd.Function):

    @staticmethod
    def forward(ctx, h, w_in, b_in, w_out, b_out):
        ext = require_ext()
        pre = F.linear(h, w_in, b_in).contiguous()
        out = F.linear(ext.gelu_fwd(pre), w_out, b_out)
        ctx.save_for_backward(h, pre, w_in, w_out)
        return out

    @staticmethod
    def backward(ctx, g):
        ext = require_ext()
        h, pre, w_in, w_out = ctx.saved_tensors
        E = h.shape[-1]
        dh, dw_in, db_in, dw_out, db_out = ext.mlp_bwd(
            g.contiguous().view(-1, E),
            h.contiguous().view(-1, E),
            pre.view(-1, pre.shape[-1]),
            w_in.contiguous(),
            w_out.contiguous(),
            _mlp_tn("in"),
            _mlp_tn("out"),
        )
        return dh.view(h.shape), dw_in, db_in, dw_out, db_out


def gptj_mlp(h, w_in, b_in, w_out, b_out):
    return _GPTJMlpFn.apply(h, w_in, b_in, w_out, b_out)


_BLOCK_SITE_DEFAULT = {
    "SAMD_ATTN_TN_QKV": True,
    "SAMD_ATTN_TN_OUT": True,
    "SAMD_DH_ACCUM": False,
}


def _block_site(name: str) -> bool:
    v = os.environ.get(name)
    return _BLOCK_SITE_DEFAULT[name] if v is None else v != "0"


def _same_tensor(a, b) -> bool:
    return (
        a.data_ptr() == b.data_ptr()
        and a.shape == b.shape
        and a.stride() == b.stride()
    )


class _GPTJBranchesFn(torch.autograd.Function):

    @staticmethod
    def forward(ctx, h, wq, wk, wv, wo, w_in, b_in, w_out, b_out, cos, sin,
                n_head, t_off):
        ext = require_ext()
        B, T, E = h.shape
        D = E // n_head
        q = F.linear(h, wq).view(B, T, n_head, D)
        k = F.linear(h, wk).view(B, T, n_head, D)
        v = F.linear(h, wv).view(B, T, n_head, D)
        qr = torch.empty_like(q)
        ext.rope_apply(qr, q, cos, sin, T, t_off, False, False)
        kr = torch.empty_like(k)
        ext.rope_apply(kr, k, cos, sin, T, t_off, False, False)
        del q, k
        qr, kr, v = qr.transpose(1, 2), kr.transpose(1, 2), v.transpose(1, 2)
        o, lse = ext.attn_fwd(qr, kr, v, True, T)
        attn_out = F.linear(o.transpose(1, 2).reshape(B, T, E), wo)
        pre = F.linear(h, w_in, b_in).contiguous()
        mlp_out = F.linear(ext.gelu_fwd(pre), w_out, b_out)
        ctx.save_for_backward(h, pre, qr, kr, v, o, lse, wq, wk, wv, wo,
                              w_in, w_out, cos, sin)
        ctx.t_off = t_off
        return attn_out, mlp_out

    @staticmethod
    def backward(ctx, g_a, g_m):
        ext = require_ext()
        (h, pre, qr, kr, v, o, lse, wq, wk, wv, wo, w_in, w_out, cos,
         sin) = ctx.saved_tensors
        E = h.shape[-1]
        if g_a is None:
            g_a = torch.zeros_like(h)
        if g_m is None:
            g_m = torch.zeros_like(h)
        if _same_tensor(g_a, g_m):
            g_a = g_m = g_m.contiguous().view(-1, E)
        else:
            g_a = g_a.contiguous().view(-1, E)
            g_m = g_m.contiguous().view(-1, E)
        dh, dwq, dwk, dwv, dwo, dw_in, db_in, dw_out, db_out = (
            ext.gptj_branches_bwd(
                g_a, g_m,
                h.contiguous().view(-1, E),
                pre.view(-1, pre.shape[-1]),
                qr, kr, v, o, lse,
                wq.contiguous(), wk.contiguous(), wv.contiguous(),
                wo.contiguous(), w_in.contiguous(), w_out.contiguous(),
                cos, sin, ctx.t_off,
                _mlp_tn("in"), _mlp_tn("out"),
                _block_site("SAMD_ATTN_TN_QKV"),
                _block_site("SAMD_ATTN_TN_OUT"),
                _block_site("SAMD_DH_ACCUM"),
            )
        )
        return (dh.view(h.shape), dwq, dwk, dwv, dwo, dw_in, db_in, dw_out,
                db_out, None, None, None, None)


def gptj_branches_supported(h, n_head, rotary_dim, table_len) -> bool:
    if h.dim() != 3 or n_head <= 0:
        return False
    B, T, E = h.shape
    if E % n_head:
        return False
    D = E // n_head
    return (
        T % 64 == 0
        and T <= table_len
        and D in (64, 128, 256)
        and rotary_dim > 0
        and rotary_dim % 8 == 0
        and rotary_dim <= D
    )


def gptj_branches(h, wq, wk, wv, wo, w_in, b_in, w_out, b_out, cos, sin,
                  n_head):
    return _GPTJBranchesFn.apply(h, wq, wk, wv, wo, w_in, b_in, w_out, b_out,
                                 cos.contiguous(), sin.contiguous(), n_head, 0)


class _SwigluFn(torch.autograd.Function):
    @staticmethod
    def forward(ctx, gate, up):
        ext = require_ext()
        gate = gate.contiguous()
        up = up.contiguous()
        ctx.save_for_backward(gate, up)
        return ext.swiglu_fwd(gate, up)

    @staticmethod
    def backward(ctx, dout):
        ext = require_ext()
        gate, up = ctx.saved_tensors
        dgate, dup = ext.swiglu_bwd(dout.contiguous(), gate, up)
        return dgate, dup


def fused_swiglu(gate, up):
    if gate.is_cuda:
        return _SwigluFn.apply(gate, up)
    return torch.nn.functional.silu(gate) * up


class _EmbedFn(torch.autograd.Function):
    @staticmethod
    def forward(ctx, weight, idx):
        ext = require_ext()
        ctx.save_for_backward(idx)
        ctx.vocab = weight.shape[0]
        return ext.embed_fwd(weight, idx)

    @staticmethod
    def backward(ctx, dout):
        ext = require_ext()
        (idx,) = ctx.saved_tensors
        return ext.embed_bwd(dout, idx, ctx.vocab), None


def fused_embedding(weight, idx):
    if weight.is_cuda:
        return _EmbedFn.apply(weight, idx)
    return F.embedding(idx, weight)


class FusedEmbedding(torch.nn.Embedding):

    def forward(self, idx):
        if (
            self.weight.is_cuda
            and self.padding_idx is None
            and self.max_norm is None
            and not self.sparse
            and self.weight.dtype
            in (torch.bfloat16, torch.float16, torch.float32)
        ):
            return _EmbedFn.apply(self.weight, idx)
        return super().forward(idx)


class _DropoutFn(torch.autograd.Function):
    @staticmethod
    def forward(ctx, x, p, seed):
        ext = require_ext()
        ctx.p = p
        ctx.seed = seed
        return ext.dropout_fwd(x, p, seed)

    @staticmethod
    def backward(ctx, dout):
        ext = require_ext()
        return ext.dropout_bwd(dout.contiguous(), ctx.p, ctx.seed), None, None


def fused_dropout(x, p: float, training: bool = True):
    if p == 0.0 or not training:
        return x
    if x.is_cuda and x.dtype in (torch.bfloat16, torch.float16):
        seed = int(torch.randint(0, 2**62, (1,)).item())
        return _DropoutFn.apply(x.contiguous(), p, seed)
    return F.dropout(x, p, training)


class FusedDropout(torch.nn.Module):
    def __init__(self, p: float = 0.0):
        super().__init__()
        self.p = p

    def forward(self, x):
        return fused_dropout(x, self.p, self.training)

    def extra_repr(self):
        return f"p={self.p}"
```

### saturn_amd/ops/optim.py

```python

from __future__ import annotations


from typing import Iterable, List, Optional

import torch

from saturn_amd.ops import require_ext


def _grouped(params_with_grads: List[torch.nn.Parameter]):
    groups = {}
    for p in params_with_grads:
        groups.setdefault((p.device, p.dtype), []).append(p)
    return groups


class FusedSGD(torch.optim.Optimizer):

    def __init__(
        self,
        params: Iterable[torch.nn.Parameter],
        lr: float,
        momentum: float = 0.0,
        weight_decay: float = 0.0,
        master_weights: bool = False,
    ) -> None:
        defaults = dict(
            lr=lr,
            momentum=momentum,
            weight_decay=weight_decay,
            master_weights=master_weights,
        )
        super().__init__(params, defaults)

    def _master_of(self, p: torch.nn.Parameter) -> Optional[torch.Tensor]:
        st = self.state[p]
        if "master" not in st:
            st["master"] = p.data.detach().to(torch.float32).contiguous()
        return st["master"]

    @torch.no_grad()
    def step(self, closure=None) -> Optional[float]:
        loss = closure() if closure is not None else None
        for group in self.param_groups:
            lr = group["lr"]
            mom = group["momentum"]
            wd = group["weight_decay"]
            use_master = group.get("master_weights", False)
            ps = [p for p in group["params"] if p.grad is not None]
            for (device, dtype), chunk in _grouped(ps).items():
                grads = [p.grad for p in chunk]
                if mom != 0.0:
                    bufs = []
                    for p in chunk:
                        st = self.state[p]
                        if "momentum_buffer" not in st:
                            st["momentum_buffer"] = torch.zeros_like(
                                p, dtype=torch.float32
                            )
                        bufs.append(st["momentum_buffer"])
                else:
                    bufs = None
                masters = None
                if use_master and dtype != torch.float32:
                    masters = [self._master_of(p) for p in chunk]
                if device.type == "cuda":
                    ext = require_ext()
                    ext.fused_sgd(
                        [p.data for p in chunk],
                        grads,
                        bufs if bufs is not None else [],
                        masters if masters is not None else [],
                        lr,
                        mom,
                        wd,
                    )
                else:
                    for i, p in enumerate(chunk):
                        g32 = grads[i].float()
                        pv = (
                            masters[i]
                            if masters is not None
                            else p.data.float()
                        )
                        if wd != 0.0:
                            g32 = g32.add(pv, alpha=wd)
                        if bufs is not None:
                            bufs[i].mul_(mom).add_(g32)
                            g32 = bufs[i]
                        nv = pv.add_(g32, alpha=-lr) if masters is not None \
                            else pv.add(g32, alpha=-lr)
                        p.data.copy_(nv.to(p.dtype))
        return loss


class FusedAdam(torch.optim.Optimizer):

    def __init__(
        self,
        params: Iterable[torch.nn.Parameter],
        lr: float = 1e-3,
        betas=(0.9, 0.999),
        eps: float = 1e-8,
        weight_decay: float = 0.0,
        master_weights: bool = False,
    ) -> None:
        defaults = dict(
            lr=lr,
            betas=betas,
            eps=eps,
            weight_decay=weight_decay,
            master_weights=master_weights,
        )
        super().__init__(params, defaults)

    @torch.no_grad()
    def step(self, closure=None) -> Optional[float]:
        loss = closure() if closure is not None else None
        for group in self.param_groups:
            lr = group["lr"]
            beta1, beta2 = group["betas"]
            eps = group["eps"]
            wd = group["weight_decay"]
            use_master = group.get("master_weights", False)
            ps = [p for p in group["params"] if p.grad is not None]
            for (device, dtype), chunk in _grouped(ps).items():
                m, v, steps = [], [], []
                masters = [] if use_master and dtype != torch.float32 else None
                for p in chunk:
                    st = self.state[p]
                    if "step" not in st:
                        st["step"] = 0
                        st["exp_avg"] = torch.zeros_like(p, dtype=torch.float32)
                        st["exp_avg_sq"] = torch.zeros_like(p, dtype=torch.float32)
                    if masters is not None and "master" not in st:
                        st["master"] = p.data.detach().to(torch.float32).contiguous()
                    st["step"] += 1
                    m.append(st["exp_avg"])
                    v.append(st["exp_avg_sq"])
                    if masters is not None:
                        masters.append(st["master"])
                    steps.append(st["step"])
                step_t = steps[0]
                bc1 = 1.0 - beta1**step_t
                bc2 = 1.0 - beta2**step_t
                grads = [p.grad for p in chunk]
                if device.type == "cuda":
                    ext = require_ext()
                    ext.fused_adam(
                        [p.data for p in chunk],
                        grads,
                        m,
                        v,
                        masters if masters is not None else [],
                        lr,
                        beta1,
                        beta2,
                        eps,
                        wd,
                        bc1,
                        bc2,
                    )
                else:
                    gf = [g.float() for g in grads]
                    torch._foreach_mul_(m, beta1)
                    torch._foreach_add_(m, gf, alpha=1 - beta1)
                    torch._foreach_mul_(v, beta2)
                    torch._foreach_addcmul_(v, gf, gf, value=1 - beta2)
                    for i, (p, mi, vi) in enumerate(zip(chunk, m, v)):
                        denom = (vi / bc2).sqrt_().add_(eps)
                        upd = (mi / bc1).div_(denom)
                        pv = masters[i] if masters is not None else p.data.float()
                        if wd != 0.0:
                            pv.mul_(1 - lr * wd)
                        pv.add_(upd, alpha=-lr)
                        p.data.copy_(pv.to(p.dtype))
        return loss
```

### saturn_amd/parallel/ddp.py

```python

from __future__ import annotations

from typing import List, Optional

import torch
import torch.distributed as dist


class _Bucket:
    def __init__(self, params: List[torch.nn.Parameter], device, dtype) -> None:
        self.params = params
        numels = [p.numel() for p in params]
        self.flat = torch.zeros(sum(numels), device=device, dtype=dtype)
        offset = 0
        self.views = []
        for p, n in zip(params, numels):
            self.views.append(self.flat[offset : offset + n].view_as(p))
            offset += n
        self.pending = 0
        self.work: Optional[dist.Work] = None
        self.launched = False

    def attach_grads(self) -> None:
        for p, v in zip(self.params, self.views):
            p.grad = v

    def reset(self) -> None:
        self.pending = len(self.params)
        self.work = None
        self.launched = False


class BucketedDDP(torch.nn.Module):

    def __init__(
        self,
        module: torch.nn.Module,
        bucket_mb: float = 64.0,
        process_group=None,
        grad_dtype: Optional[torch.dtype] = None,
        comm=None,
        exclude=None,
        use_buckets: Optional[bool] = None,
    ) -> None:
        super().__init__()
        self.module = module
        self.pg = process_group
        self.comm = comm
        if comm is not None:
            self.world = comm.world
        else:
            self.world = (
                dist.get_world_size(process_group) if dist.is_initialized() else 1
            )

        skip = {id(p) for p in (exclude or ())}
        if self.world > 1:
            with torch.no_grad():
                if comm is not None:
                    for p in module.parameters():
                        if id(p) not in skip:
                            comm.broadcast(p.data, 0)
                    comm.join()
                else:
                    for p in module.parameters():
                        if id(p) not in skip:
                            dist.broadcast(p.data, src=0, group=self.pg)

        params = [
            p for p in module.parameters()
            if p.requires_grad and id(p) not in skip
        ]
        self.buckets: List[_Bucket] = []
        self._param_bucket = {}
        if use_buckets is None:
            use_buckets = self.world > 1
        if not use_buckets:
            return
        bucket_bytes = int(bucket_mb * 1024 * 1024)
        cur: List[torch.nn.Parameter] = []
        cur_bytes = 0
        for p in reversed(params):
            if cur and (
                cur_bytes + p.numel() * p.element_size() > bucket_bytes
                or p.dtype != cur[0].dtype
                or p.device != cur[0].device
            ):
                self._seal(cur, grad_dtype)
                cur, cur_bytes = [], 0
            cur.append(p)
            cur_bytes += p.numel() * p.element_size()
        if cur:
            self._seal(cur, grad_dtype)

        for b in self.buckets:
            b.attach_grads()
            b.reset()
            for p in b.params:
                self._param_bucket[p] = b
                p.register_post_accumulate_grad_hook(self._hook)

    def _seal(self, params: List[torch.nn.Parameter], grad_dtype) -> None:
        p0 = params[0]
        self.buckets.append(
            _Bucket(params, p0.device, grad_dtype or p0.dtype)
        )

    def _launch(self, b: _Bucket) -> None:
        if self.comm is not None:
            self.comm.all_reduce(b.flat, True)
            b.launched = True
        else:
            b.work = dist.all_reduce(b.flat, async_op=True, group=self.pg)

    def _hook(self, p: torch.nn.Parameter) -> None:
        b = self._param_bucket[p]
        b.pending -= 1
        if b.pending == 0 and self.world > 1:
            self._launch(b)

    def forward(self, *args, **kwargs):
        return self.module(*args, **kwargs)

    def grad_sync(self) -> None:
        if self.world > 1:
            for b in self.buckets:
                launched = (
                    b.launched if self.comm is not None else b.work is not None
                )
                if not launched:
                    self._launch(b)
        if self.comm is not None:
            if self.world > 1:
                self.comm.join()
            for b in self.buckets:
                b.reset()
            return
        inv = 1.0 / self.world
        for b in self.buckets:
            if b.work is not None:
                b.work.wait()
            if self.world > 1:
                b.flat.mul_(inv)
            b.reset()

    def zero_grad_buffers(self, set_to_none: bool = False) -> None:
        if not self.buckets:
            self.module.zero_grad(set_to_none=True)
            return
        for b in self.buckets:
            b.flat.zero_()
            b.attach_grads()
            b.reset()
```

### saturn_amd/parallel/tensor.py

```python

from __future__ import annotations



import torch
import torch.distributed as dist
import torch.nn as nn


def _world() -> int:
    return dist.get_world_size() if dist.is_initialized() else 1


def _rank() -> int:
    return dist.get_rank() if dist.is_initialized() else 0


class _CopyToTP(torch.autograd.Function):

    @staticmethod
    def forward(ctx, x):
        return x

    @staticmethod
    def backward(ctx, g):
        if _world() > 1:
            g = g.contiguous()
            dist.all_reduce(g)
        return g


class _ReduceFromTP(torch.autograd.Function):

    @staticmethod
    def forward(ctx, x):
        if _world() > 1:
            x = x.contiguous()
            dist.all_reduce(x)
        return x

    @staticmethod
    def backward(ctx, g):
        return g


class ColumnParallelLinear(nn.Module):

    def __init__(self, linear: nn.Linear):
        super().__init__()
        w, r = _world(), _rank()
        out_f, in_f = linear.weight.shape
        assert out_f % w == 0, f"out_features {out_f} % tp {w} != 0"
        sl = slice(r * out_f // w, (r + 1) * out_f // w)
        self.weight = nn.Parameter(linear.weight.data[sl].clone())
        self.bias = (
            nn.Parameter(linear.bias.data[sl].clone())
            if linear.bias is not None
            else None
        )
        self.full_out = out_f

    def forward(self, x):
        return torch.nn.functional.linear(_CopyToTP.apply(x), self.weight, self.bias)


class RowParallelLinear(nn.Module):

    def __init__(self, linear: nn.Linear):
        super().__init__()
        w, r = _world(), _rank()
        out_f, in_f = linear.weight.shape
        assert in_f % w == 0, f"in_features {in_f} % tp {w} != 0"
        sl = slice(r * in_f // w, (r + 1) * in_f // w)
        self.weight = nn.Parameter(linear.weight.data[:, sl].clone())
        self.bias = (
            nn.Parameter(linear.bias.data.clone())
            if linear.bias is not None
            else None
        )

    def forward(self, x_local):
        y = torch.nn.functional.linear(x_local, self.weight)
        y = _ReduceFromTP.apply(y)
        if self.bias is not None:
            y = y + self.bias
        return y


def tp_shard_model(model: nn.Module) -> nn.Module:
    from saturn_amd.models.gptj import GPTJBlock
    from saturn_amd.models.llama import LlamaBlock

    w = _world()
    if w == 1:
        return model
    for m in model.modules():
        if isinstance(m, GPTJBlock):
            a = m.attn
            assert a.n_head % w == 0
            a.q_proj = ColumnParallelLinear(a.q_proj)
            a.k_proj = ColumnParallelLinear(a.k_proj)
            a.v_proj = ColumnParallelLinear(a.v_proj)
            a.out_proj = RowParallelLinear(a.out_proj)
            a.n_head //= w
            m.mlp.fc_in = ColumnParallelLinear(m.mlp.fc_in)
            m.mlp.fc_out = RowParallelLinear(m.mlp.fc_out)
        elif isinstance(m, LlamaBlock):
            a = m.self_attn
            assert a.n_head % w == 0 and a.n_kv % w == 0
            a.q_proj = ColumnParallelLinear(a.q_proj)
            a.k_proj = ColumnParallelLinear(a.k_proj)
            a.v_proj = ColumnParallelLinear(a.v_proj)
            a.o_proj = RowParallelLinear(a.o_proj)
            a.n_head //= w
            a.n_kv //= w
            m.mlp.gate_proj = ColumnParallelLinear(m.mlp.gate_proj)
            m.mlp.up_proj = ColumnParallelLinear(m.mlp.up_proj)
            m.mlp.down_proj = RowParallelLinear(m.mlp.down_proj)
    return model


def tp_replicated_parameters(model: nn.Module):
    sharded = set()
    for mod in model.modules():
        if isinstance(mod, ColumnParallelLinear):
            sharded.add(id(mod.weight))
            if mod.bias is not None:
                sharded.add(id(mod.bias))
        elif isinstance(mod, RowParallelLinear):
            sharded.add(id(mod.weight))
    return [p for p in model.parameters() if id(p) not in sharded]


@torch.no_grad()
def tp_resync_replicated(model: nn.Module) -> None:
    if _world() == 1:
        return
    for p in tp_replicated_parameters(model):
        dist.broadcast(p.data, src=0)


@torch.no_grad()
def tp_full_state_dict(model: nn.Module):
    w = _world()
    if w == 1:
        return {k: v.cpu().clone() for k, v in model.state_dict().items()}
    full = {}
    for name, mod in model.named_modules():
        if isinstance(mod, ColumnParallelLinear):
            shards = [torch.empty_like(mod.weight) for _ in range(w)]
            dist.all_gather(shards, mod.weight.data.contiguous())
            full[f"{name}.weight"] = torch.cat(shards, dim=0).cpu()
            if mod.bias is not None:
                bs = [torch.empty_like(mod.bias) for _ in range(w)]
                dist.all_gather(bs, mod.bias.data.contiguous())
                full[f"{name}.bias"] = torch.cat(bs, dim=0).cpu()
        elif isinstance(mod, RowParallelLinear):
            shards = [torch.empty_like(mod.weight) for _ in range(w)]
            dist.all_gather(shards, mod.weight.data.contiguous())
            full[f"{name}.weight"] = torch.cat(shards, dim=1).cpu()
            if mod.bias is not None:
                full[f"{name}.bias"] = mod.bias.data.cpu().clone()
    sd = model.state_dict()
    out = {}
    for k, v in sd.items():
        hit = None
        for fk in full:
            if k == fk or k.endswith("." + fk):
                hit = full[fk]
                break
        out[k] = hit if hit is not None else v.cpu().clone()
    return out if _rank() == 0 else None
```

### saturn_amd/parallel/zero3.py

```python

from __future__ import annotations

import logging
from typing import Dict, List, Optional, Sequence

import torch
import torch.distributed as dist
import torch.nn as nn

log = logging.getLogger(__name__)


def _world() -> int:
    return dist.get_world_size() if dist.is_initialized() else 1


def _rank() -> int:
    return dist.get_rank() if dist.is_initialized() else 0


def _allgather_into(full: torch.Tensor, shard: torch.Tensor, async_op=False):
    if _world() == 1:
        full.copy_(shard)
        return None
    if dist.get_backend() == "gloo":
        chunks = list(full.chunk(_world()))
        return dist.all_gather(chunks, shard, async_op=async_op)
    return dist.all_gather_into_tensor(full, shard, async_op=async_op)


def _reducescatter_into(shard: torch.Tensor, full: torch.Tensor):
    if _world() == 1:
        shard.copy_(full)
        return
    if dist.get_backend() == "gloo":
        dist.all_reduce(full)
        shard.copy_(full.chunk(_world())[_rank()])
        return
    dist.reduce_scatter_tensor(shard, full)


_copy_streams: Dict[int, "torch.cuda.Stream"] = {}


def _copy_stream(device) -> Optional["torch.cuda.Stream"]:
    if device.type != "cuda":
        return None
    idx = device.index or 0
    if idx not in _copy_streams:
        _copy_streams[idx] = torch.cuda.Stream(device=device)
    return _copy_streams[idx]


class _Unit:

    def __init__(self, idx: int, module: nn.Module, params: List[nn.Parameter],
                 device, offload: bool) -> None:
        self.idx = idx
        self.module = module
        self.params = params
        self.device = device
        self.offload = offload
        world = _world()
        numel = sum(p.numel() for p in params)
        self.pad_numel = (numel + world - 1) // world * world
        self.shard_numel = self.pad_numel // world
        dtype = params[0].dtype
        self.dtype = dtype

        flat = torch.zeros(self.pad_numel, dtype=dtype, device=device)
        offset = 0
        self.offsets: List[int] = []
        self.shapes: List[torch.Size] = []
        self.numels: List[int] = []
        for p in params:
            flat[offset : offset + p.numel()].copy_(p.data.view(-1))
            self.offsets.append(offset)
            self.shapes.append(p.shape)
            self.numels.append(p.numel())
            offset += p.numel()
        r = _rank()
        shard = flat[r * self.shard_numel : (r + 1) * self.shard_numel].clone()
        if offload:
            host = torch.empty(
                shard.shape, dtype=shard.dtype, device="cpu",
                pin_memory=device.type == "cuda",
            )
            host.copy_(shard)
            shard = host
        self.shard = nn.Parameter(shard)
        del flat
        self._placeholder = torch.empty(0, dtype=dtype, device=device)
        for p in params:
            p.data = self._placeholder
        self.full: Optional[torch.Tensor] = None
        self.gathered = False
        self.work = None
        self.copy_event: Optional["torch.cuda.Event"] = None
        self.grad_pending = 0

    def _materialize_full(self) -> torch.Tensor:
        if self.full is None:
            self.full = torch.empty(
                self.pad_numel, dtype=self.dtype, device=self.device
            )
        elif self.full.untyped_storage().size() == 0:
            self.full.untyped_storage().resize_(
                self.pad_numel * self.full.element_size()
            )
        return self.full

    def start_gather(self, async_op: bool = False) -> None:
        if self.gathered:
            return
        self.gathered = True
        full = self._materialize_full()
        cs = _copy_stream(self.device) if self.offload else None
        if cs is not None:
            full.record_stream(cs)
            ev = torch.cuda.Event()
            with torch.cuda.stream(cs):
                shard_dev = self.shard.data.to(self.device, non_blocking=True)
                if _world() == 1:
                    full.copy_(shard_dev)
                    self.work = None
                else:
                    self.work = _allgather_into(
                        full, shard_dev, async_op=async_op
                    )
                ev.record(cs)
            self.copy_event = ev
            return
        shard_dev = self.shard.data
        self.work = _allgather_into(full, shard_dev, async_op=async_op)

    def finish_gather(self) -> None:
        if self.copy_event is not None:
            torch.cuda.current_stream(self.device).wait_event(self.copy_event)
            self.copy_event = None
        if self.work is not None:
            self.work.wait()
            self.work = None
        for p, off, shp, n in zip(self.params, self.offsets, self.shapes, self.numels):
            p.data = self.full[off : off + n].view(shp)

    def free(self) -> None:
        for p in self.params:
            p.data = self._placeholder
        if self.copy_event is not None:
            self.copy_event.synchronize()
            self.copy_event = None
        if self.work is not None:
            self.work.wait()
        if self.full is not None and self.gathered:
            self.full.untyped_storage().resize_(0)
        self.gathered = False
        self.work = None

    def reduce_grads(self) -> None:
        full_grad = torch.zeros(
            self.pad_numel, dtype=self.dtype, device=self.device
        )
        for p, off, n in zip(self.params, self.offsets, self.numels):
            if p.grad is not None:
                full_grad[off : off + n].copy_(p.grad.view(-1))
                p.grad = None
        grad_shard = torch.empty(
            self.shard_numel, dtype=self.dtype, device=self.device
        )
        _reducescatter_into(grad_shard, full_grad)
        if _world() > 1:
            grad_shard.div_(_world())
        if self.offload:
            grad_shard = grad_shard.to("cpu")
        if self.shard.grad is None:
            self.shard.grad = grad_shard
        else:
            self.shard.grad.add_(grad_shard)


class Zero3Model(nn.Module):

    def __init__(
        self,
        model: nn.Module,
        unit_modules: Optional[Sequence[nn.Module]] = None,
        device: Optional[torch.device] = None,
        offload: bool = False,
        checkpoint_activations: bool = False,
        prefetch: bool = True,
    ) -> None:
        super().__init__()
        self.model = model
        self.device = device or next(model.parameters()).device
        self.checkpoint_activations = checkpoint_activations
        self.prefetch = prefetch and self.device.type == "cuda"

        if unit_modules is None:
            if hasattr(model, "h"):
                unit_modules = list(model.h)
            else:
                unit_modules = [
                    m for m in model.children() if any(p.requires_grad for p in m.parameters())
                ]
        unit_modules = list(unit_modules)

        if _world() > 1:
            with torch.no_grad():
                for p in model.parameters():
                    dist.broadcast(p.data, src=0)

        claimed = set()
        self.units: List[_Unit] = []
        for i, m in enumerate(unit_modules):
            ps = [p for p in m.parameters() if p.requires_grad]
            self.units.append(_Unit(i, m, ps, self.device, offload))
            claimed |= {id(p) for p in ps}
        rest = [
            p for p in model.parameters() if p.requires_grad and id(p) not in claimed
        ]
        if rest:
            self.units.append(
                _Unit(len(self.units), model, rest, self.device, offload)
            )
        self._unit_of_module: Dict[int, _Unit] = {
            id(u.module): u for u in self.units
        }
        self._install_hooks()

    @staticmethod
    def _triggers(u: _Unit) -> List[nn.Module]:
        m = u.module
        if isinstance(m, (nn.ModuleList, nn.ModuleDict)):
            return list(m.children())
        return [m]

    def _install_hooks(self) -> None:
        for u in self.units:
            if u.module is self.model:
                continue
            triggers = self._triggers(u)
            for t in triggers:
                t.register_forward_pre_hook(self._fwd_pre(u))
                t.register_full_backward_pre_hook(self._bwd_pre(u))
            triggers[-1].register_forward_hook(self._fwd_post(u))
            for p in u.params:
                p.register_post_accumulate_grad_hook(self._grad_hook(u))

    def _fwd_pre(self, u: _Unit):
        def hook(module, args):
            u.start_gather()
            u.finish_gather()
            if self.prefetch and u.idx + 1 < len(self.units):
                nxt = self.units[u.idx + 1]
                if nxt.module is not self.model:
                    nxt.start_gather(async_op=True)
        return hook

    def _fwd_post(self, u: _Unit):
        def hook(module, args, output):
            u.free()
        return hook

    def _bwd_pre(self, u: _Unit):
        def hook(module, grad_output):
            u.start_gather()
            u.finish_gather()
            if u.grad_pending == 0:
                u.grad_pending = len(u.params)
            if self.prefetch and u.idx - 1 >= 0:
                prv = self.units[u.idx - 1]
                if prv.module is not self.model:
                    prv.start_gather(async_op=True)
        return hook

    def _grad_hook(self, u: _Unit):
        def hook(p):
            u.grad_pending -= 1
            if u.grad_pending == 0:
                u.reduce_grads()
                u.free()
        return hook

    def forward(self, *args, **kwargs):
        res = self.units[-1]
        if res.module is self.model:
            res.start_gather()
            res.finish_gather()
            res.grad_pending = len(res.params)
        if self.checkpoint_activations:
            out = self._forward_with_checkpointing(*args, **kwargs)
        else:
            out = self.model(*args, **kwargs)
        return out

    def _forward_with_checkpointing(self, *args, **kwargs):
        from torch.utils.checkpoint import checkpoint

        m = self.model
        if not hasattr(m, "wte") or not hasattr(m, "h"):
            return m(*args, **kwargs)
        x = args[0]
        h = m.wte(x)
        if hasattr(m, "wpe"):
            pos = torch.arange(x.shape[1], device=x.device)
            h = h + m.wpe(pos)[None]
        for blk in m.h:
            h = checkpoint(blk, h, use_reentrant=False)
        h = m.ln_f(h)
        return m.lm_head(h)

    def grad_sync(self) -> None:
        res = self.units[-1]
        if res.module is self.model and res.gathered:
            res.reduce_grads()
            res.free()

    def sharded_parameters(self) -> List[nn.Parameter]:
        return [u.shard for u in self.units]

    def zero_grad_shards(self) -> None:
        for u in self.units:
            u.shard.grad = None

    @torch.no_grad()
    def full_state_dict(self) -> Optional[Dict[str, torch.Tensor]]:
        for u in self.units:
            u.start_gather()
            u.finish_gather()
        sd = None
        if _rank() == 0:
            sd = {k: v.detach().cpu().clone() for k, v in self.model.state_dict().items()}
        for u in self.units:
            u.free()
        return sd
```

### saturn_amd/utils/graph_step.py

```python

from __future__ import annotations

from typing import Callable, Optional

import torch


class GraphedStep:

    def __init__(
        self,
        step_fn: Callable[[], torch.Tensor],
        warmup: int = 3,
        stream: Optional[torch.cuda.Stream] = None,
    ):
        assert torch.cuda.is_available(), "GraphedStep needs a GPU"
        self._graph = torch.cuda.CUDAGraph()
        s = stream or torch.cuda.Stream()
        s.wait_stream(torch.cuda.current_stream())
        with torch.cuda.stream(s):
            for _ in range(max(1, warmup)):
                step_fn()
        torch.cuda.current_stream().wait_stream(s)
        torch.cuda.synchronize()
        with torch.cuda.graph(self._graph):
            self.loss = step_fn()

    def replay(self) -> torch.Tensor:
        self._graph.replay()
        return self.loss


def graphed_train_step(model, loss_fn, optimizer, example_input, ddp=None,
                       warmup: int = 3) -> tuple:
    static_x = example_input.clone()

    def step():
        if ddp is not None:
            ddp.zero_grad_buffers()
        else:
            optimizer.zero_grad(set_to_none=False)
        logits = model(static_x) if ddp is None else ddp(static_x)
        loss = loss_fn(logits, static_x)
        loss.backward()
        if ddp is not None:
            ddp.grad_sync()
        optimizer.step()
        return loss

    return GraphedStep(step, warmup=warmup), static_x
```

Before: 61.56 samples/s.

## Maintain transposed weight shadows in fused SGD for TN input-gradient GEMMs

Adds a fused SGD kernel that, after updating each large 2-D bf16 weight, also writes a transposed copy into a per-parameter shadow buffer. The GPT-J MLP and branch backward kernels can then take W^T and run their input-gradient GEMMs in the TN layout instead of the slower layout. Shadows are versioned, invalidated on broadcasts, sharding, Adam and graph capture. The cost is an extra weight-sized bf16 buffer per large matrix and extra transposed writes in the optimizer step.

```diff
diff --git a/saturn_amd/executors/megatron.py b/saturn_amd/executors/megatron.py
--- a/saturn_amd/executors/megatron.py
+++ b/saturn_amd/executors/megatron.py
@@ -5,6 +5,7 @@
 from typing import Any, Dict, List, Optional, Tuple
 
 from saturn_amd.core.technique import BaseTechnique
+from saturn_amd.ops import wt_shadow
 from saturn_amd.executors.launch import (
     destroy_process_group,
     gang_spawn,
@@ -40,6 +41,7 @@
             with torch.no_grad():
                 for p in model.parameters():
                     dist.broadcast(p.data, src=0)
+                    wt_shadow.invalidate(p)
         model = tp_shard_model(model)
         optimizer = _make_optimizer(task, model)
 
diff --git a/saturn_amd/models/gptj.py b/saturn_amd/models/gptj.py
--- a/saturn_amd/models/gptj.py
+++ b/saturn_amd/models/gptj.py
@@ -22,7 +22,9 @@
     mlp_fused_supported,
     gptj_branches,
     gptj_branches_supported,
+    dgrad_tn_site,
 )
+from saturn_amd.ops import wt_shadow
 
 
 @dataclass
@@ -73,6 +75,12 @@
         return self.out_proj(o)
 
 
+def _request_shadows(sites) -> None:
+    for site, w in sites:
+        if dgrad_tn_site(site):
+            wt_shadow.request(w)
+
+
 class GPTJMLP(nn.Module):
     def __init__(self, cfg: GPTJConfig):
         super().__init__()
@@ -103,6 +111,8 @@
     def forward(self, x):
         if self._use_fused(x):
             fi, fo = self.fc_in, self.fc_out
+            if self.training:
+                _request_shadows((("IN", fi.weight), ("OUT", fo.weight)))
             return gptj_mlp(x, fi.weight, fi.bias, fo.weight, fo.bias)
         return self.fc_out(fused_gelu(self.fc_in(x)))
 
@@ -162,6 +172,13 @@
         if self._use_fused(h):
             attn, mlp = self.attn, self.mlp
             cos, sin = attn._rope(h.device)
+            if self.training:
+                _request_shadows((
+                    ("PROJ", attn.q_proj.weight), ("PROJ", attn.k_proj.weight),
+                    ("PROJ", attn.v_proj.weight),
+                    ("PROJ", attn.out_proj.weight),
+                    ("IN", mlp.fc_in.weight), ("OUT", mlp.fc_out.weight),
+                ))
             a, m = gptj_branches(
                 h, attn.q_proj.weight, attn.k_proj.weight, attn.v_proj.weight,
                 attn.out_proj.weight, mlp.fc_in.weight, mlp.fc_in.bias,
diff --git a/saturn_amd/ops/csrc/bindings.cpp b/saturn_amd/ops/csrc/bindings.cpp
--- a/saturn_amd/ops/csrc/bindings.cpp
+++ b/saturn_amd/ops/csrc/bindings.cpp
@@ -6,6 +6,10 @@
 void fused_sgd(std::vector<at::Tensor> params, std::vector<at::Tensor> grads,
                std::vector<at::Tensor> moms, std::vector<at::Tensor> masters,
                double lr, double momentum, double weight_decay);
+void fused_sgd_t(std::vector<at::Tensor> params, std::vector<at::Tensor> grads,
+                 std::vector<at::Tensor> moms, std::vector<at::Tensor> masters,
+                 std::vector<at::Tensor> shadows, double lr, double momentum,
+                 double weight_decay);
 void fused_adam(std::vector<at::Tensor> params, std::vector<at::Tensor> grads,
                 std::vector<at::Tensor> ms, std::vector<at::Tensor> vs,
                 std::vector<at::Tensor> masters, double lr, double beta1,
@@ -54,7 +58,9 @@
 std::vector<at::Tensor> transpose_colsum(at::Tensor x, bool want_sum);
 std::vector<at::Tensor> mlp_bwd(at::Tensor g, at::Tensor h, at::Tensor pre,
                                 at::Tensor W_in, at::Tensor W_out,
-                                bool use_tn_in, bool use_tn_out);
+                                bool use_tn_in, bool use_tn_out,
+                                c10::optional<at::Tensor> W_inT,
+                                c10::optional<at::Tensor> W_outT);
 void transpose_into(at::Tensor x, at::Tensor dst);
 at::Tensor rope_bwd_t(at::Tensor dy, at::Tensor cos_t, at::Tensor sin_t,
                       int64_t t_len, int64_t t_off, int64_t dim,
@@ -64,12 +70,18 @@
     at::Tensor k, at::Tensor v, at::Tensor o, at::Tensor lse, at::Tensor Wq,
     at::Tensor Wk, at::Tensor Wv, at::Tensor Wo, at::Tensor W_in,
     at::Tensor W_out, at::Tensor cos_t, at::Tensor sin_t, int64_t t_off,
-    bool tn_in, bool tn_out, bool tn_qkv, bool tn_o, bool dh_accum);
+    bool tn_in, bool tn_out, bool tn_qkv, bool tn_o, bool dh_accum,
+    c10::optional<at::Tensor> WqT, c10::optional<at::Tensor> WkT,
+    c10::optional<at::Tensor> WvT, c10::optional<at::Tensor> WoT,
+    c10::optional<at::Tensor> W_inT, c10::optional<at::Tensor> W_outT);
 }
 
 PYBIND11_MODULE(TORCH_EXTENSION_NAME, m) {
   m.doc() = "saturn_amd hand-written CDNA4 (gfx950) kernels";
   m.def("fused_sgd", &samd::fused_sgd, "fused multi-tensor SGD");
+  m.def("fused_sgd_t", &samd::fused_sgd_t,
+        "fused multi-tensor SGD for 2-D bf16 params that also stores each "
+        "updated param transposed into its [C, R] shadow");
   m.def("fused_adam", &samd::fused_adam, "fused multi-tensor AdamW");
   m.def("norm_fwd", &samd::norm_fwd, "LayerNorm/RMSNorm forward");
   m.def("norm_bwd", &samd::norm_bwd, "LayerNorm/RMSNorm backward");
@@ -116,7 +128,11 @@
   m.def("transpose_colsum", &samd::transpose_colsum,
         "bf16 transpose with optional fp32 column sums");
   m.def("mlp_bwd", &samd::mlp_bwd,
-        "GPT-J MLP backward with TN-layout weight gradients");
+        "GPT-J MLP backward with TN-layout weight gradients; with W^T given "
+        "the input gradients run as TN GEMMs too",
+        py::arg("g"), py::arg("h"), py::arg("pre"), py::arg("W_in"),
+        py::arg("W_out"), py::arg("use_tn_in"), py::arg("use_tn_out"),
+        py::arg("W_inT") = py::none(), py::arg("W_outT") = py::none());
   m.def("transpose_into", &samd::transpose_into,
         "bf16 transpose stored into a caller-given [N, M] view",
         py::arg("x"), py::arg("dst"));
@@ -125,5 +141,15 @@
         py::arg("dy"), py::arg("cos"), py::arg("sin"), py::arg("t_len"),
         py::arg("t_off"), py::arg("dim"), py::arg("dxT"));
   m.def("gptj_branches_bwd", &samd::gptj_branches_bwd,
-        "GPT-J attention + MLP branch backward with shared transposes");
+        "GPT-J attention + MLP branch backward with shared transposes; with "
+        "W^T given the input gradients run as TN GEMMs too",
+        py::arg("g_a"), py::arg("g_m"), py::arg("h"), py::arg("pre"),
+        py::arg("q"), py::arg("k"), py::arg("v"), py::arg("o"), py::arg("lse"),
+        py::arg("Wq"), py::arg("Wk"), py::arg("Wv"), py::arg("Wo"),
+        py::arg("W_in"), py::arg("W_out"), py::arg("cos"), py::arg("sin"),
+        py::arg("t_off"), py::arg("tn_in"), py::arg("tn_out"),
+        py::arg("tn_qkv"), py::arg("tn_o"), py::arg("dh_accum"),
+        py::arg("WqT") = py::none(), py::arg("WkT") = py::none(),
+        py::arg("WvT") = py::none(), py::arg("WoT") = py::none(),
+        py::arg("W_inT") = py::none(), py::arg("W_outT") = py::none());
 }
diff --git a/saturn_amd/ops/csrc/fused_optim.hip b/saturn_amd/ops/csrc/fused_optim.hip
--- a/saturn_amd/ops/csrc/fused_optim.hip
+++ b/saturn_amd/ops/csrc/fused_optim.hip
@@ -4,6 +4,7 @@
 #include <vector>
 
 #include "common.h"
+#include "tile_image.h"
 
 namespace samd {
 
@@ -38,6 +39,34 @@
   float nv = pv - a.lr * gv;
   if (HAS_W) w[j] = nv;
   p[j] = fromF<T>(nv);
+}
+
+template <typename T, bool HAS_M, bool HAS_W>
+__device__ __forceinline__ void sgd_update8(short8v_& pv, const short8v_& gv,
+                                            float4v_& m0, float4v_& m1,
+                                            float4v_& w0, float4v_& w1,
+                                            float lr, float momentum,
+                                            float weight_decay) {
+#pragma unroll
+  for (int e = 0; e < GRP; ++e) {
+    T pe, ge;
+    pe.x = (unsigned short)pv[e];
+    ge.x = (unsigned short)gv[e];
+    float pf = HAS_W ? (e < 4 ? w0[e] : w1[e - 4]) : toF<T>(pe);
+    float gf = toF<T>(ge);
+    if (weight_decay != 0.f) gf += weight_decay * pf;
+    if (HAS_M) {
+      float mv = (e < 4 ? m0[e] : m1[e - 4]) * momentum + gf;
+      if (e < 4) m0[e] = mv; else m1[e - 4] = mv;
+      gf = mv;
+    }
+    float nf = pf - lr * gf;
+    if (HAS_W) {
+      if (e < 4) w0[e] = nf; else w1[e - 4] = nf;
+    }
+    T out = fromF<T>(nf);
+    pv[e] = (short)out.x;
+  }
 }
 
 template <typename T, bool HAS_M, bool HAS_W>
@@ -70,26 +99,8 @@
           w0 = *reinterpret_cast<float4v_*>(w + base);
           w1 = *reinterpret_cast<float4v_*>(w + base + 4);
         }
-#pragma unroll
-        for (int e = 0; e < GRP; ++e) {
-          T pe, ge;
-          pe.x = (unsigned short)pv[e];
-          ge.x = (unsigned short)gv[e];
-          float pf = HAS_W ? (e < 4 ? w0[e] : w1[e - 4]) : toF<T>(pe);
-          float gf = toF<T>(ge);
-          if (a.weight_decay != 0.f) gf += a.weight_decay * pf;
-          if (HAS_M) {
-            float mv = (e < 4 ? m0[e] : m1[e - 4]) * a.momentum + gf;
-            if (e < 4) m0[e] = mv; else m1[e - 4] = mv;
-            gf = mv;
-          }
-          float nf = pf - a.lr * gf;
-          if (HAS_W) {
-            if (e < 4) w0[e] = nf; else w1[e - 4] = nf;
-          }
-          T out = fromF<T>(nf);
-          pv[e] = (short)out.x;
-        }
+        sgd_update8<T, HAS_M, HAS_W>(pv, gv, m0, m1, w0, w1, a.lr, a.momentum,
+                                     a.weight_decay);
         *reinterpret_cast<short8v_*>(p + base) = pv;
         if (HAS_M) {
           *reinterpret_cast<float4v_*>(m + base) = m0;
@@ -108,6 +119,104 @@
       for (long j = base; j < end; ++j)
         sgd_elem<T, HAS_M, HAS_W>(p, g, m, w, j, a);
     }
+  }
+}
+
+struct SgdTArgs {
+  void* p[MAX_T];
+  void* g[MAX_T];
+  void* m[MAX_T];
+  void* w[MAX_T];
+  void* pT[MAX_T];
+  long cum[MAX_T + 1];
+  long rows[MAX_T];
+  long cols[MAX_T];
+  int n_tensors;
+  float lr, momentum, weight_decay;
+};
+
+template <bool HAS_M, bool HAS_W>
+__global__ void __launch_bounds__(MB_BLOCK) fused_sgd_t_kernel(SgdTArgs a) {
+  __shared__ uint4 img[MB_TILE * 8];
+
+  const long i = blockIdx.x;
+  int t = 0;
+#pragma unroll
+  for (int k = 0; k < MAX_T; ++k)
+    if (k < a.n_tensors && i >= a.cum[k + 1]) t = k + 1;
+  const long R = a.rows[t], C = a.cols[t];
+  const long gx = (C + MB_TILE - 1) / MB_TILE;
+  const long u = i - a.cum[t];
+  const long bx = u % gx, by = u / gx;
+  bf16_t* p = reinterpret_cast<bf16_t*>(a.p[t]);
+  const bf16_t* g = reinterpret_cast<const bf16_t*>(a.g[t]);
+  float* m = HAS_M ? reinterpret_cast<float*>(a.m[t]) : nullptr;
+  float* w = HAS_W ? reinterpret_cast<float*>(a.w[t]) : nullptr;
+  bf16_t* pT = reinterpret_cast<bf16_t*>(a.pT[t]);
+
+  const int tid = threadIdx.x;
+  const int cv = tid & 7;
+  const int rp = tid >> 3;
+  const int mv = tid & 7;
+  const int cr = tid >> 3;
+  const long col0 = bx * MB_TILE;
+  const long col = col0 + cv * 8;
+  const bool col_ok = col < C;
+
+  for (int it = 0; it < MB_ROW_ITERS; ++it) {
+    const long row0 = (by * MB_ROW_ITERS + it) * MB_TILE;
+    if (row0 >= R) break;
+    const long row = row0 + 2 * rp;
+    const bool ok = col_ok && row < R;
+
+    const short8v_ zero8 = {0, 0, 0, 0, 0, 0, 0, 0};
+    short8v_ pv[2];
+#pragma unroll
+    for (int r = 0; r < 2; ++r) {
+      pv[r] = zero8;
+      if (!ok) continue;
+      const long o = (row + r) * C + col;
+      pv[r] = *reinterpret_cast<const short8v_*>(p + o);
+      const short8v_ gv = *reinterpret_cast<const short8v_*>(g + o);
+      float4v_ m0, m1, w0, w1;
+      if (HAS_M) {
+        m0 = *reinterpret_cast<float4v_*>(m + o);
+        m1 = *reinterpret_cast<float4v_*>(m + o + 4);
+      }
+      if (HAS_W) {
+        w0 = *reinterpret_cast<float4v_*>(w + o);
+        w1 = *reinterpret_cast<float4v_*>(w + o + 4);
+      }
+      sgd_update8<bf16_t, HAS_M, HAS_W>(pv[r], gv, m0, m1, w0, w1, a.lr,
+                                        a.momentum, a.weight_decay);
+      *reinterpret_cast<short8v_*>(p + o) = pv[r];
+      if (HAS_M) {
+        *reinterpret_cast<float4v_*>(m + o) = m0;
+        *reinterpret_cast<float4v_*>(m + o + 4) = m1;
+      }
+      if (HAS_W) {
+        *reinterpret_cast<float4v_*>(w + o) = w0;
+        *reinterpret_cast<float4v_*>(w + o + 4) = w1;
+      }
+    }
+    unsigned* i32 = reinterpret_cast<unsigned*>(img);
+#pragma unroll
+    for (int e = 0; e < 8; ++e) {
+      i32[img_dword(cv * 8 + e, rp)] =
+          (unsigned)(unsigned short)pv[0][e] |
+          ((unsigned)(unsigned short)pv[1][e] << 16);
+    }
+    __syncthreads();
+
+    const long mrow = row0 + mv * 8;
+#pragma unroll
+    for (int j = 0; j < 2; ++j) {
+      const int c = cr + 32 * j;
+      if ((col0 + c < C) && (mrow < R))
+        *reinterpret_cast<uint4*>(pT + (col0 + c) * R + mrow) =
+            img[img_slot(c, mv)];
+    }
+    __syncthreads();
   }
 }
 
@@ -299,6 +408,84 @@
       break;
     default:
       TORCH_CHECK(false, "fused_sgd: unsupported dtype");
+  }
+}
+
+void fused_sgd_t(std::vector<at::Tensor> params, std::vector<at::Tensor> grads,
+                 std::vector<at::Tensor> moms, std::vector<at::Tensor> masters,
+                 std::vector<at::Tensor> shadows, double lr, double momentum,
+                 double weight_decay) {
+  TORCH_CHECK(!params.empty(), "no params");
+  TORCH_CHECK(params.size() == grads.size() &&
+              params.size() == shadows.size());
+  TORCH_CHECK(moms.empty() || moms.size() == params.size());
+  TORCH_CHECK(masters.empty() || masters.size() == params.size());
+  const auto fp32_like = [](const at::Tensor& t, const at::Tensor& p) {
+    return t.is_cuda() && t.scalar_type() == at::kFloat && t.is_contiguous() &&
+           t.sizes() == p.sizes() && t.device() == p.device() &&
+           reinterpret_cast<uintptr_t>(t.data_ptr()) % 16 == 0;
+  };
+  for (size_t i = 0; i < params.size(); ++i) {
+    const at::Tensor& p = params[i];
+    check_operand(p, "fused_sgd_t param");
+    check_operand(grads[i], "fused_sgd_t grad");
+    check_operand(shadows[i], "fused_sgd_t shadow");
+    TORCH_CHECK(grads[i].sizes() == p.sizes() &&
+                    grads[i].device() == p.device(),
+                "fused_sgd_t: grad does not match its param");
+    TORCH_CHECK(shadows[i].size(0) == p.size(1) &&
+                    shadows[i].size(1) == p.size(0) &&
+                    shadows[i].device() == p.device(),
+                "fused_sgd_t: shadow must be [", p.size(1), ", ", p.size(0),
+                "], got ", shadows[i].sizes());
+    if (!moms.empty())
+      TORCH_CHECK(fp32_like(moms[i], p),
+                  "momentum buffers must be contiguous fp32 like the param");
+    if (!masters.empty())
+      TORCH_CHECK(fp32_like(masters[i], p),
+                  "master weights must be contiguous fp32 like the param");
+  }
+  auto stream = at::hip::getCurrentHIPStream();
+  const bool has_m = !moms.empty();
+  const bool has_w = !masters.empty();
+  for (size_t base = 0; base < params.size(); base += MAX_T) {
+    SgdTArgs a{};
+    a.n_tensors = (int)std::min<size_t>(MAX_T, params.size() - base);
+    a.lr = (float)lr;
+    a.momentum = (float)momentum;
+    a.weight_decay = (float)weight_decay;
+    long cum = 0;
+    a.cum[0] = 0;
+    for (int k = 0; k < a.n_tensors; ++k) {
+      const at::Tensor& p = params[base + k];
+      a.p[k] = p.data_ptr();
+      a.g[k] = grads[base + k].data_ptr();
+      a.m[k] = has_m ? moms[base + k].data_ptr() : nullptr;
+      a.w[k] = has_w ? masters[base + k].data_ptr() : nullptr;
+      a.pT[k] = shadows[base + k].data_ptr();
+      a.rows[k] = p.size(0);
+      a.cols[k] = p.size(1);
+      const long gx = (a.cols[k] + MB_TILE - 1) / MB_TILE;
+      const long gy = (a.rows[k] + MB_TILE * MB_ROW_ITERS - 1) /
+                      (MB_TILE * MB_ROW_ITERS);
+      cum += gx * gy;
+      a.cum[k + 1] = cum;
+    }
+    TORCH_CHECK(cum <= 0x7fffffffL, "fused_sgd_t: too many tiles");
+    const dim3 grid((unsigned)cum);
+    if (has_m && has_w)
+      hipLaunchKernelGGL((fused_sgd_t_kernel<true, true>), grid,
+                         dim3(MB_BLOCK), 0, stream.stream(), a);
+    else if (has_m)
+      hipLaunchKernelGGL((fused_sgd_t_kernel<true, false>), grid,
+                         dim3(MB_BLOCK), 0, stream.stream(), a);
+    else if (has_w)
+      hipLaunchKernelGGL((fused_sgd_t_kernel<false, true>), grid,
+                         dim3(MB_BLOCK), 0, stream.stream(), a);
+    else
+      hipLaunchKernelGGL((fused_sgd_t_kernel<false, false>), grid,
+                         dim3(MB_BLOCK), 0, stream.stream(), a);
+    SAMD_CHECK_HIP(hipGetLastError());
   }
 }
 
diff --git a/saturn_amd/ops/csrc/gptj_block_bwd.hip b/saturn_amd/ops/csrc/gptj_block_bwd.hip
--- a/saturn_amd/ops/csrc/gptj_block_bwd.hip
+++ b/saturn_amd/ops/csrc/gptj_block_bwd.hip
@@ -147,7 +147,10 @@
     at::Tensor k, at::Tensor v, at::Tensor o, at::Tensor lse, at::Tensor Wq,
     at::Tensor Wk, at::Tensor Wv, at::Tensor Wo, at::Tensor W_in,
     at::Tensor W_out, at::Tensor cos_t, at::Tensor sin_t, int64_t t_off,
-    bool tn_in, bool tn_out, bool tn_qkv, bool tn_o, bool dh_accum) {
+    bool tn_in, bool tn_out, bool tn_qkv, bool tn_o, bool dh_accum,
+    c10::optional<at::Tensor> WqT, c10::optional<at::Tensor> WkT,
+    c10::optional<at::Tensor> WvT, c10::optional<at::Tensor> WoT,
+    c10::optional<at::Tensor> W_inT, c10::optional<at::Tensor> W_outT) {
   check_operand(g_a, "gptj_branches_bwd g_a");
   check_operand(g_m, "gptj_branches_bwd g_m");
   check_operand(h, "gptj_branches_bwd h");
@@ -169,6 +172,13 @@
     TORCH_CHECK(w->size(0) == E && w->size(1) == E,
                 "gptj_branches_bwd: projection weights must be [E, E]");
   }
+  const at::Tensor wqT = checked_wt(WqT, Wq, "gptj_branches_bwd WqT");
+  const at::Tensor wkT = checked_wt(WkT, Wk, "gptj_branches_bwd WkT");
+  const at::Tensor wvT = checked_wt(WvT, Wv, "gptj_branches_bwd WvT");
+  const at::Tensor woT = checked_wt(WoT, Wo, "gptj_branches_bwd WoT");
+  const at::Tensor w_inT = checked_wt(W_inT, W_in, "gptj_branches_bwd W_inT");
+  const at::Tensor w_outT =
+      checked_wt(W_outT, W_out, "gptj_branches_bwd W_outT");
   auto o_phys = o.permute({0, 2, 1, 3});
   TORCH_CHECK(o_phys.is_contiguous(),
               "gptj_branches_bwd: o must be physically [B,T,H,D]");
@@ -185,7 +195,7 @@
   {
     at::Tensor d_pre, d_preT, act;
     {
-      auto d_act = at::mm(g_m, W_out);
+      auto d_act = dgrad(g_m, W_out, w_outT);
       auto r = mlp_act_bwd(d_act, pre, tn_in, tn_out);
       d_pre = r[0];
       d_preT = r[1];
@@ -198,10 +208,10 @@
     dW_in = tn_in ? at::linear(d_preT, hT) : at::mm(d_pre.t(), h);
     d_preT.reset();
     if (!tn_qkv) hT.reset();
-    dh = at::mm(d_pre, W_in);
-  }
-
-  auto d_o = at::mm(g_a, Wo);
+    dh = dgrad(d_pre, W_in, w_inT);
+  }
+
+  auto d_o = dgrad(g_a, Wo, woT);
   at::Tensor dWo;
   if (tn_o) {
     auto oT = transpose_colsum_impl(o2, false, true)[0];
@@ -254,13 +264,13 @@
 
   auto dq2 = dq.view({M, E}), dk2 = dk.view({M, E});
   if (dh_accum) {
-    dh.addmm_(dv2, Wv);
-    dh.addmm_(dk2, Wk);
-    dh.addmm_(dq2, Wq);
+    dh.addmm_(dv2, wvT.defined() ? wvT.t() : Wv);
+    dh.addmm_(dk2, wkT.defined() ? wkT.t() : Wk);
+    dh.addmm_(dq2, wqT.defined() ? wqT.t() : Wq);
   } else {
-    dh.add_(at::mm(dv2, Wv));
-    dh.add_(at::mm(dk2, Wk));
-    dh.add_(at::mm(dq2, Wq));
+    dh.add_(dgrad(dv2, Wv, wvT));
+    dh.add_(dgrad(dk2, Wk, wkT));
+    dh.add_(dgrad(dq2, Wq, wqT));
   }
   return {dh, dWq, dWk, dWv, dWo, dW_in, db_in.to(W_in.scalar_type()),
           dW_out, gt[1].to(W_out.scalar_type())};
diff --git a/saturn_amd/ops/csrc/mlp_bwd.hip b/saturn_amd/ops/csrc/mlp_bwd.hip
--- a/saturn_amd/ops/csrc/mlp_bwd.hip
+++ b/saturn_amd/ops/csrc/mlp_bwd.hip
@@ -238,7 +238,9 @@
 
 std::vector<at::Tensor> mlp_bwd(at::Tensor g, at::Tensor h, at::Tensor pre,
                                 at::Tensor W_in, at::Tensor W_out,
-                                bool use_tn_in, bool use_tn_out) {
+                                bool use_tn_in, bool use_tn_out,
+                                c10::optional<at::Tensor> W_inT,
+                                c10::optional<at::Tensor> W_outT) {
   check_operand(g, "mlp_bwd g");
   check_operand(h, "mlp_bwd h");
   check_operand(pre, "mlp_bwd pre");
@@ -249,10 +251,12 @@
                   W_in.size(0) == F && W_in.size(1) == E &&
                   W_out.size(0) == E && W_out.size(1) == F,
               "mlp_bwd: inconsistent shapes");
+  const at::Tensor w_inT = checked_wt(W_inT, W_in, "mlp_bwd W_inT");
+  const at::Tensor w_outT = checked_wt(W_outT, W_out, "mlp_bwd W_outT");
 
   at::Tensor d_pre, d_preT, act, db_in;
   {
-    auto d_act = at::mm(g, W_out);
+    auto d_act = dgrad(g, W_out, w_outT);
     auto r = mlp_act_bwd(d_act, pre, use_tn_in, use_tn_out);
     d_pre = r[0];
     d_preT = r[1];
@@ -267,7 +271,7 @@
   auto dW_in = use_tn_in ? at::linear(d_preT, hT) : at::mm(d_pre.t(), h);
   d_preT.reset();
   hT.reset();
-  auto dh = at::mm(d_pre, W_in);
+  auto dh = dgrad(d_pre, W_in, w_inT);
   return {dh, dW_in, db_in.to(W_in.scalar_type()), dW_out,
           gt[1].to(W_out.scalar_type())};
 }
diff --git a/saturn_amd/ops/csrc/tile_image.h b/saturn_amd/ops/csrc/tile_image.h
--- a/saturn_amd/ops/csrc/tile_image.h
+++ b/saturn_amd/ops/csrc/tile_image.h
@@ -68,6 +68,22 @@
               ": data must be 16-byte aligned");
 }
 
+inline at::Tensor checked_wt(const c10::optional<at::Tensor>& WT,
+                             const at::Tensor& W, const char* name) {
+  if (!WT.has_value() || !WT->defined()) return at::Tensor();
+  check_operand(*WT, name);
+  TORCH_CHECK(WT->size(0) == W.size(1) && WT->size(1) == W.size(0) &&
+                  WT->device() == W.device(),
+              name, ": expected [", W.size(1), ", ", W.size(0), "], got ",
+              WT->sizes());
+  return *WT;
+}
+
+inline at::Tensor dgrad(const at::Tensor& dY, const at::Tensor& W,
+                        const at::Tensor& WT) {
+  return WT.defined() ? at::linear(dY, WT) : at::mm(dY, W);
+}
+
 inline dim3 tile_grid(long M, long N) {
   const long gx = (N + MB_TILE - 1) / MB_TILE;
   const long gy = (M + MB_TILE * MB_ROW_ITERS - 1) / (MB_TILE * MB_ROW_ITERS);
diff --git a/saturn_amd/ops/functional.py b/saturn_amd/ops/functional.py
--- a/saturn_amd/ops/functional.py
+++ b/saturn_amd/ops/functional.py
@@ -7,7 +7,7 @@
 import torch
 import torch.nn.functional as F
 
-from saturn_amd.ops import require_ext
+from saturn_amd.ops import require_ext, wt_shadow
 
 
 class _NormFn(torch.autograd.Function):
@@ -320,6 +320,7 @@
         pre = F.linear(h, w_in, b_in).contiguous()
         out = F.linear(ext.gelu_fwd(pre), w_out, b_out)
         ctx.save_for_backward(h, pre, w_in, w_out)
+        ctx.weights = (w_in, w_out)
         return out
 
     @staticmethod
@@ -335,6 +336,8 @@
             w_out.contiguous(),
             _mlp_tn("in"),
             _mlp_tn("out"),
+            _wt("IN", ctx.weights[0]),
+            _wt("OUT", ctx.weights[1]),
         )
         return dh.view(h.shape), dw_in, db_in, dw_out, db_out
 
@@ -347,12 +350,23 @@
     "SAMD_ATTN_TN_QKV": True,
     "SAMD_ATTN_TN_OUT": True,
     "SAMD_DH_ACCUM": False,
+    "SAMD_DGRAD_TN_PROJ": False,
+    "SAMD_DGRAD_TN_IN": True,
+    "SAMD_DGRAD_TN_OUT": True,
 }
 
 
 def _block_site(name: str) -> bool:
     v = os.environ.get(name)
     return _BLOCK_SITE_DEFAULT[name] if v is None else v != "0"
+
+
+def dgrad_tn_site(site: str) -> bool:
+    return _block_site("SAMD_DGRAD_TN_" + site)
+
+
+def _wt(site: str, w):
+    return wt_shadow.get(w) if dgrad_tn_site(site) else None
 
 
 def _same_tensor(a, b) -> bool:
@@ -387,6 +401,7 @@
         ctx.save_for_backward(h, pre, qr, kr, v, o, lse, wq, wk, wv, wo,
                               w_in, w_out, cos, sin)
         ctx.t_off = t_off
+        ctx.weights = (wq, wk, wv, wo, w_in, w_out)
         return attn_out, mlp_out
 
     @staticmethod
@@ -417,6 +432,9 @@
                 _block_site("SAMD_ATTN_TN_QKV"),
                 _block_site("SAMD_ATTN_TN_OUT"),
                 _block_site("SAMD_DH_ACCUM"),
+                *(_wt(site, w) for site, w in zip(
+                    ("PROJ", "PROJ", "PROJ", "PROJ", "IN", "OUT"),
+                    ctx.weights)),
             )
         )
         return (dh.view(h.shape), dwq, dwk, dwv, dwo, dw_in, db_in, dw_out,
diff --git a/saturn_amd/ops/optim.py b/saturn_amd/ops/optim.py
--- a/saturn_amd/ops/optim.py
+++ b/saturn_amd/ops/optim.py
@@ -6,7 +6,7 @@
 
 import torch
 
-from saturn_amd.ops import require_ext
+from saturn_amd.ops import require_ext, wt_shadow
 
 
 def _grouped(params_with_grads: List[torch.nn.Parameter]):
@@ -14,6 +14,15 @@
     for p in params_with_grads:
         groups.setdefault((p.device, p.dtype), []).append(p)
     return groups
+
+
+def _shadow_for(p: torch.nn.Parameter) -> Optional[torch.Tensor]:
+    g = p.grad
+    if not (g.dtype == p.dtype and g.is_contiguous()
+            and g.data_ptr() % 16 == 0):
+        wt_shadow.invalidate(p)
+        return None
+    return wt_shadow.maintain(p)
 
 
 class FusedSGD(torch.optim.Optimizer):
@@ -65,17 +74,26 @@
                 masters = None
                 if use_master and dtype != torch.float32:
                     masters = [self._master_of(p) for p in chunk]
+                shadows = [_shadow_for(p) for p in chunk]
                 if device.type == "cuda":
                     ext = require_ext()
-                    ext.fused_sgd(
-                        [p.data for p in chunk],
-                        grads,
-                        bufs if bufs is not None else [],
-                        masters if masters is not None else [],
-                        lr,
-                        mom,
-                        wd,
-                    )
+                    for want in (False, True):
+                        idx = [i for i, s in enumerate(shadows)
+                               if (s is not None) == want]
+                        if not idx:
+                            continue
+                        args = (
+                            [chunk[i].data for i in idx],
+                            [grads[i] for i in idx],
+                            [bufs[i] for i in idx] if bufs is not None else [],
+                            [masters[i] for i in idx]
+                            if masters is not None else [],
+                        )
+                        if want:
+                            ext.fused_sgd_t(*args, [shadows[i] for i in idx],
+                                            lr, mom, wd)
+                        else:
+                            ext.fused_sgd(*args, lr, mom, wd)
                 else:
                     for i, p in enumerate(chunk):
                         g32 = grads[i].float()
@@ -92,6 +110,11 @@
                         nv = pv.add_(g32, alpha=-lr) if masters is not None \
                             else pv.add(g32, alpha=-lr)
                         p.data.copy_(nv.to(p.dtype))
+                        if shadows[i] is not None:
+                            shadows[i].copy_(p.data.t())
+                for p, s in zip(chunk, shadows):
+                    if s is not None:
+                        wt_shadow.commit(p)
         return loss
 
 
@@ -146,6 +169,7 @@
                 bc1 = 1.0 - beta1**step_t
                 bc2 = 1.0 - beta2**step_t
                 grads = [p.grad for p in chunk]
+                wt_shadow.invalidate_all(chunk)
                 if device.type == "cuda":
                     ext = require_ext()
                     ext.fused_adam(
diff --git a/saturn_amd/ops/wt_shadow.py b/saturn_amd/ops/wt_shadow.py
--- /dev/null
+++ b/saturn_amd/ops/wt_shadow.py
@@ -0,0 +1,103 @@
+
+from __future__ import annotations
+
+import contextlib
+import os
+from typing import Optional
+
+import torch
+
+MIN_DIM = 1024
+
+_REQ = "_samd_wt_requested"
+_SHADOW = "_samd_wt_shadow"
+
+
+def min_dim() -> int:
+    v = os.environ.get("SAMD_WT_MIN_DIM")
+    return MIN_DIM if v is None else int(v)
+
+
+_suspended = 0
+
+
+@contextlib.contextmanager
+def suspend():
+    global _suspended
+    _suspended += 1
+    try:
+        yield
+    finally:
+        _suspended -= 1
+
+
+def _capturing() -> bool:
+    return _suspended > 0 or (
+        torch.cuda.is_available() and torch.cuda.is_current_stream_capturing()
+    )
+
+
+def request(p: torch.Tensor) -> None:
+    setattr(p, _REQ, True)
+
+
+def requested(p: torch.Tensor) -> bool:
+    return getattr(p, _REQ, False)
+
+
+def has_shadow(p: torch.Tensor) -> bool:
+    return getattr(p, _SHADOW, None) is not None
+
+
+def eligible(p: torch.Tensor) -> bool:
+    if not requested(p) or p.dim() != 2 or p.dtype != torch.bfloat16:
+        return False
+    r, c = p.shape
+    d = min_dim()
+    return (
+        r >= d and c >= d and r % 8 == 0 and c % 8 == 0
+        and p.is_contiguous() and p.data_ptr() % 16 == 0
+    )
+
+
+def maintain(p: torch.Tensor) -> Optional[torch.Tensor]:
+    if _capturing():
+        invalidate(p)
+        return None
+    if not eligible(p):
+        if has_shadow(p):
+            invalidate(p)
+        return None
+    rec = getattr(p, _SHADOW, None)
+    want = (p.shape[1], p.shape[0])
+    if rec is None or tuple(rec[0].shape) != want or rec[0].device != p.device:
+        buf = torch.empty(want, dtype=p.dtype, device=p.device)
+    else:
+        buf = rec[0]
+    setattr(p, _SHADOW, (buf, None, None))
+    return buf
+
+
+def commit(p: torch.Tensor) -> None:
+    rec = getattr(p, _SHADOW)
+    setattr(p, _SHADOW, (rec[0], p._version, p.data_ptr()))
+
+
+def get(p: torch.Tensor) -> Optional[torch.Tensor]:
+    rec = getattr(p, _SHADOW, None)
+    if rec is None or _capturing():
+        return None
+    buf, version, ptr = rec
+    if version != p._version or ptr != p.data_ptr():
+        return None
+    return buf
+
+
+def invalidate(p: torch.Tensor) -> None:
+    if getattr(p, _SHADOW, None) is not None:
+        setattr(p, _SHADOW, None)
+
+
+def invalidate_all(params) -> None:
+    for p in params:
+        invalidate(p)
diff --git a/saturn_amd/parallel/ddp.py b/saturn_amd/parallel/ddp.py
--- a/saturn_amd/parallel/ddp.py
+++ b/saturn_amd/parallel/ddp.py
@@ -5,6 +5,8 @@
 
 import torch
 import torch.distributed as dist
+
+from saturn_amd.ops import wt_shadow
 
 
 class _Bucket:
@@ -61,11 +63,13 @@
                     for p in module.parameters():
                         if id(p) not in skip:
                             comm.broadcast(p.data, 0)
+                            wt_shadow.invalidate(p)
                     comm.join()
                 else:
                     for p in module.parameters():
                         if id(p) not in skip:
                             dist.broadcast(p.data, src=0, group=self.pg)
+                            wt_shadow.invalidate(p)
 
         params = [
             p for p in module.parameters()
diff --git a/saturn_amd/parallel/tensor.py b/saturn_amd/parallel/tensor.py
--- a/saturn_amd/parallel/tensor.py
+++ b/saturn_amd/parallel/tensor.py
@@ -6,6 +6,8 @@
 import torch
 import torch.distributed as dist
 import torch.nn as nn
+
+from saturn_amd.ops import wt_shadow
 
 
 def _world() -> int:
@@ -138,6 +140,7 @@
         return
     for p in tp_replicated_parameters(model):
         dist.broadcast(p.data, src=0)
+        wt_shadow.invalidate(p)
 
 
 @torch.no_grad()
diff --git a/saturn_amd/parallel/zero3.py b/saturn_amd/parallel/zero3.py
--- a/saturn_amd/parallel/zero3.py
+++ b/saturn_amd/parallel/zero3.py
@@ -7,6 +7,8 @@
 import torch
 import torch.distributed as dist
 import torch.nn as nn
+
+from saturn_amd.ops import wt_shadow
 
 log = logging.getLogger(__name__)
 
@@ -93,6 +95,7 @@
         self._placeholder = torch.empty(0, dtype=dtype, device=device)
         for p in params:
             p.data = self._placeholder
+            wt_shadow.invalidate(p)
         self.full: Optional[torch.Tensor] = None
         self.gathered = False
         self.work = None
@@ -209,6 +212,7 @@
             with torch.no_grad():
                 for p in model.parameters():
                     dist.broadcast(p.data, src=0)
+                    wt_shadow.invalidate(p)
 
         claimed = set()
         self.units: List[_Unit] = []
diff --git a/saturn_amd/utils/graph_step.py b/saturn_amd/utils/graph_step.py
--- a/saturn_amd/utils/graph_step.py
+++ b/saturn_amd/utils/graph_step.py
@@ -4,6 +4,8 @@
 from typing import Callable, Optional
 
 import torch
+
+from saturn_amd.ops import wt_shadow
 
 
 class GraphedStep:
@@ -18,13 +20,14 @@
         self._graph = torch.cuda.CUDAGraph()
         s = stream or torch.cuda.Stream()
         s.wait_stream(torch.cuda.current_stream())
-        with torch.cuda.stream(s):
-            for _ in range(max(1, warmup)):
-                step_fn()
-        torch.cuda.current_stream().wait_stream(s)
-        torch.cuda.synchronize()
-        with torch.cuda.graph(self._graph):
-            self.loss = step_fn()
+        with wt_shadow.suspend():
+            with torch.cuda.stream(s):
+                for _ in range(max(1, warmup)):
+                    step_fn()
+            torch.cuda.current_stream().wait_stream(s)
+            torch.cuda.synchronize()
+            with torch.cuda.graph(self._graph):
+                self.loss = step_fn()
 
     def replay(self) -> torch.Tensor:
         self._graph.replay()
```

After: 62.66 samples/s, median of 6. 1.02x the previous value.
